# abalakrishna123/recovery-rl

Measured on AMD Instinct MI355X. Metric: env-steps/sec + SAC grad-steps/sec, Navigation1 4096 envs, 1/2/4/8 GPU, higher is better.
Workload: dtype f32

## Files before the change

include/rrl_hip.h:

```cpp
#ifndef RRL_HIP_H
#define RRL_HIP_H

#include <stdint.h>

#ifdef __cplusplus
extern "C" {
#endif

#define RRL_OK 0
#define RRL_EINVAL (-1)
#define RRL_ELAUNCH (-2)
#define RRL_ECAPTURE (-5)
#define RRL_EPLANS (-6)
#define RRL_ERANGE (-3)

enum { RRL_ENV_NAV1 = 0, RRL_ENV_NAV2 = 1, RRL_ENV_MAZE = 2 };

enum {
    RRL_STREAM_STEP = 0,
    RRL_STREAM_RESET = 1,
    RRL_STREAM_OFFLINE = 2,
    RRL_STREAM_SAMPLE = 3,
    RRL_STREAM_SAMPLE_NEG = 4,
    RRL_STREAM_CEM = 5,
// ... 181 lines not shown
    uint8_t* active;
    float* action;
} rrl_cem_set_t;
int rrl_cem_begin(const rrl_cem_set_t* s, void* stream);
int rrl_cem_finish(const rrl_cem_set_t* s, void* stream);

int rrl_gemm_f32(int mode, int G, int M, int N, int K, const float* A, int lda, long long sA,
                 const float* B, int ldb, long long sB, float* C, int ldc, long long sC,
                 const float* bias, long long sBias, int relu, const float* mask, int ldmask,
                 long long sMask, float* colsum, long long sColsum, int accumulate, void* stream);

int rrl_mlp3_forward(int G, int M, int H, int din, int dout, const float* x, int ldx, const float* W1,
                     const float* b1, const float* W2, const float* b2, const float* W3, const float* b3,
                     float* h1, float* h2, float* out, float* scratch, int finalize, void* stream);
int rrl_mlp3_is_split(int M, int H);

enum { RRL_LOSS_SAC_CRITIC = 0, RRL_LOSS_SAC_POLICY = 1, RRL_LOSS_QRISK_CRITIC = 2, RRL_LOSS_QRISK_POLICY = 3,
       RRL_LOSS_GAUSS_HEAD = 4, RRL_LOSS_STOCH_HEAD = 5, RRL_LOSS_DGD_QRISK = 6 };
typedef struct {
    int kind;
    int n_part;
    long long part_stride;
    const float *out, *out_t;
    const float *v0, *v1, *v2, *v3;
    const float* alpha;
    float f0;
    int ld, n_heads;
    long long head_stride;
    const float* d_action;
    float* loss;
    int da_parts;
    long long da_part_stride;
    int da_group;
} rrl_loss_t;

typedef struct {
    int G, M, H, din, dout, ldx;
    const float *x, *W1, *b1, *W2, *b2, *W3, *b3;
    float *h1, *h2, *out, *scratch;
    rrl_policy_head_t in_head;
    int use_in_head;
    const float* W2p;
} rrl_stack_t;
typedef struct {
    rrl_loss_t loss;
    int G, B, H, dout;
    const float *h2, *W3;
    float *dW3, *db3;
    float* dh2;
} rrl_head_bwd_t;
typedef struct {
    const float *x, *W1;
    int ldx, din;
    float* first_part;
    long long first_stride;
    float* dx_part;
    int dx_fold;
} rrl_first_layer_t;
typedef struct {
    int G, B, H;
    const float *dh2, *h1, *W2;
    float *dW2, *db2;
    float* dh1;
    rrl_first_layer_t first;
} rrl_hidden_bwd_t;
typedef struct {
    int G, B, H, din, ldx;
    const float *dh1, *x, *W1;
    float *dW1, *db1;
    float* dx;
} rrl_input_bwd_t;
int rrl_mlp3_forward_multi(int n, const rrl_stack_t* stacks, void* stream);
typedef struct {
    const rrl_draw_ahead_t* select;
    const rrl_draw_ahead_t* gather;
    const rrl_draw_t* second;
    long long noise_pairs;
    uint64_t noise_seed, noise_counter;
    uint64_t* noise_counter_dev;
    uint64_t noise_counter_inc;
    float* noise_out;
} rrl_fwd_riders_t;
int rrl_mlp3_forward_riders(const rrl_stack_t* stack, const rrl_fwd_riders_t* riders, void* stream);
int rrl_mlp_head_backward_multi(int n, const rrl_head_bwd_t* members, void* stream);
int rrl_mlp_hidden_backward_multi(int n, const rrl_hidden_bwd_t* members, void* stream);
int rrl_mlp_input_backward_multi(int n, const rrl_input_bwd_t* members, void* stream);
int rrl_mlp_backward_pair_multi(int n, const rrl_head_bwd_t* heads, const rrl_hidden_bwd_t* hidden, void* stream);

int rrl_loss_dout(const rrl_loss_t* loss, int B, float* dout, void* stream);
typedef struct {
    int B;
    const float* z;
    int n_part;
    long long part_stride;
    const float* lambda;
    float* penalty;
    float* mean;
} rrl_penalty_args_t;
int rrl_rcpo_penalty(const rrl_penalty_args_t* a, void* stream);
int rrl_policy_heads_fwd_multi(int n, const rrl_policy_head_t* heads, void* stream);
#define RRL_ADAM_MAX_SEGS 12
typedef struct {
    long long n;
    float* p;
    const float* g;
    float* m;
    float* v;
    uint64_t* step_dev;
    float* target;
    float tau;
    float weight_decay;
    const float* g2;
    const float* g_part;
    int n_part;
    long long part_stride, part_elems;
    float* w2p;
    float* target_w2p;
    long long w2_off;
    int w2_heads;
} rrl_adam_seg_t;
int rrl_adam_step_multi(int n_seg, const rrl_adam_seg_t* segs, float lr, float beta1, float beta2, float eps,
                        void* stream);
#define RRL_ADAM_MAX_DUALS 4
typedef struct {
    float *log_p, *exp_avg, *exp_avg_sq, *step;
    float* value;
    const float* stat;
    float eps_safe;
    float lr;
    const float* loss_in;
    float* loss_out;
    float f_loss;
} rrl_dual_t;
int rrl_adam_step_multi_duals(int n_seg, const rrl_adam_seg_t* segs, int n_dual, const rrl_dual_t* duals, float lr,
                              float beta1, float beta2, float eps, void* stream);
int rrl_w2_pack(int G, int H, const float* W2, float* W2p, void* stream);
int rrl_normal_fill(long long n_pairs, uint64_t seed, uint64_t counter, uint64_t* counter_dev, uint64_t counter_inc,
                    float* out, void* stream);
int rrl_recovery_select(int N, const float* z, float eps_safe, const float* task_action, int ld_task,
                        const float* rec_action, float* real_action, uint8_t* recovery, float* task_out,
                        void* stream);

#define RRL_EPLOG_I32 6
typedef struct {
    int32_t* rec_i32;
    double* rec_f64;
    int64_t cap;
    int64_t* state;
} rrl_episode_log_t;

int rrl_episode_log_append(int64_t n, const float* reward, const uint8_t* constraint, const uint8_t* success,
                           const uint8_t* ep_done, const uint8_t* recovery, int32_t* ep_len, double* ep_ret,
                           int32_t* ep_viol, int32_t* ep_rec, const rrl_episode_log_t* log, void* stream);

typedef struct {
    int hq, he, n_nets;
    const float *q_w1, *q_b1, *q_w2, *q_b2, *q_w3, *q_b3;
    const float *e_w0, *e_b0, *e_w1, *e_b1, *e_w2, *e_b2, *e_w3, *e_b3;
    const float *inputs_mu, *inputs_sigma, *max_logvar, *min_logvar;
} rrl_plan_weights_t;

int rrl_plan_supported(int hq, int he, int n_nets, int npart, int d_obs, int d_act);
long long rrl_plan_pack_floats(int hq, int he, int n_nets);
long long rrl_plan_scratch_floats(int n_nets, long long M, int pop);
int rrl_plan_pack(const rrl_plan_weights_t* w, int f16x3, float* packed, void* stream);
typedef struct {
    const float* packed;
    int hq, he, n_nets, npart;
    int f16x3;
    long long M;
// ... 195 lines not shown
```

recovery_rl_amd/_lib.py:

```python
import ctypes as C
import os
import subprocess

_HERE = os.path.dirname(os.path.abspath(__file__))
CSRC = os.path.join(_HERE, "csrc")
SO_PATH = os.environ.get("RRL_HIP_LIB") or os.path.join(CSRC, "librrl_hip.so")
INCLUDE = os.path.join(os.path.dirname(_HERE), "include")

HIP_SOURCES = ["nav_kernels.hip", "replay_kernels.hip", "maze_kernels.hip", "cem_kernels.hip",
               "mlp_kernels.hip", "mlp_fwd_kernels.hip", "update_kernels.hip", "log_kernels.hip", "plan_kernels.hip", "ens_train_kernels.hip",
               "ens_train_big_kernels.hip", "sqrl_kernels.hip", "qsample_kernels.hip", "eval_kernels.hip",
               "sqrl_f16x3_kernels.hip", "qsample_f16x3_kernels.hip"]
HIPCC_FLAGS = ["--offload-arch=gfx950", "-O3", "-std=c++17", "-fPIC", "-shared",
               "-ffp-contract=off", "-Wall", "-Wno-unused-function",
               "-Wno-bitwise-instead-of-logical"]

SOURCE_FLAGS = {
    "nav_kernels.hip": ["-mllvm", "-amdgpu-atomic-optimizer-strategy=None"],
    "maze_kernels.hip": ["-mllvm", "-amdgpu-atomic-optimizer-strategy=None"],
    "update_kernels.hip": ["-mllvm", "-amdgpu-atomic-optimizer-strategy=None"],
}

EXPORTS = [
    "rrl_abi_version", "rrl_last_hip_error", "rrl_counter_add",
    "rrl_nav_step", "rrl_nav_step_compact", "rrl_nav_reset", "rrl_nav_rollout", "rrl_nav_offline_rollouts",
    "rrl_nav_offline",
    "rrl_maze_step", "rrl_maze_reset", "rrl_maze_offline",
    "rrl_replay_push", "rrl_sample_multi", "rrl_draw_select", "rrl_mlp3_forward_riders",
    "rrl_nav_step_push_x", "rrl_maze_step_push_x",
    "rrl_sample_multi_packed", "rrl_pack_clear", "rrl_mlp3_forward_multi_packed", "rrl_mlp_head_backward_multi_packed",
    "rrl_mlp_hidden_backward_multi_packed", "rrl_mlp_backward_pair_multi_packed", "rrl_adam_step_multi_packed", "rrl_nav_step_push_packed",
    "rrl_maze_step_push_packed",
    "rrl_adam_step_multi_duals_packed", "rrl_rcpo_penalty_packed", "rrl_policy_heads_fwd_multi_packed",
    "rrl_cem_sample", "rrl_cem_update", "rrl_cem_begin", "rrl_cem_finish",
    "rrl_gemm_f32", "rrl_mlp3_forward", "rrl_mlp3_is_split",
    "rrl_mlp3_forward_multi", "rrl_mlp_head_backward_multi", "rrl_mlp_hidden_backward_multi",
    "rrl_mlp_input_backward_multi", "rrl_mlp_backward_pair_multi", "rrl_policy_heads_fwd_multi",
    "rrl_loss_dout", "rrl_rcpo_penalty", "rrl_adam_step_multi_duals",
    "rrl_adam_step_multi", "rrl_w2_pack", "rrl_normal_fill", "rrl_recovery_select", "rrl_episode_log_append",
    "rrl_plan_supported", "rrl_plan_pack_floats", "rrl_plan_scratch_floats", "rrl_plan_pack", "rrl_plan_cost",
    "rrl_ens_train_supported", "rrl_ens_scratch_floats", "rrl_ens_train_grad", "rrl_ens_train_epoch",
    "rrl_ens_train_big_supported", "rrl_ens_big_scratch_floats", "rrl_ens_train_grad_big", "rrl_ens_train_epoch_big",
    "rrl_sqrl_scratch_floats", "rrl_sqrl_act", "rrl_sqrl_act_packed",
    "rrl_qsample_scratch_floats", "rrl_qsample_act", "rrl_qsample_act_gated", "rrl_qsample_act_packed",
    "rrl_eval_rollout", "rrl_eval_rollout_packed", "rrl_eval_rollout_maze", "rrl_eval_rollout_maze_packed",
    "rrl_eval_rollout_qs", "rrl_eval_rollout_qs_packed",
    "rrl_eval_rollout_sqrl", "rrl_eval_rollout_sqrl_packed",
    "rrl_w2_pack_f16x3", "rrl_sqrl_act_f16x3", "rrl_sqrl_act_f16x3_packed",
    "rrl_qsample_act_f16x3", "rrl_qsample_act_gated_f16x3", "rrl_qsample_act_f16x3_packed",
    "rrl_eval_rollout_qs_f16x3", "rrl_eval_rollout_qs_f16x3_packed",
    "rrl_eval_rollout_sqrl_f16x3", "rrl_eval_rollout_sqrl_f16x3_packed",
]

class RRLError(RuntimeError):
    pass


def _sources():
    return [os.path.join(CSRC, f) for f in HIP_SOURCES if os.path.exists(os.path.join(CSRC, f))]


def _stale():
    if not os.path.exists(SO_PATH):
        return True
    t = os.path.getmtime(SO_PATH)
    deps = _sources() + [os.path.join(CSRC, f) for f in os.listdir(CSRC) if f.endswith(".hpp")]
    deps.append(os.path.join(INCLUDE, "rrl_hip.h"))
    return any(os.path.getmtime(d) > t for d in deps)


_FLAG_PROBES = {}


def flags_supported(hipcc, flags):
    key = (hipcc,) + tuple(flags)
    if key not in _FLAG_PROBES:
        import tempfile
        with tempfile.TemporaryDirectory() as tmp:
            src = os.path.join(tmp, "probe.hip")
            open(src, "w").write("// empty\n")
            r = subprocess.run([hipcc, "--offload-arch=gfx950", "-c", "-o", os.path.join(tmp, "probe.o"), src] + list(flags),
                               capture_output=True)
            _FLAG_PROBES[key] = r.returncode == 0
    return _FLAG_PROBES[key]


def build(force=False, verbose=False, jobs=None):
    if not force and not _stale():
        return SO_PATH
    from concurrent.futures import ThreadPoolExecutor
    hipcc = os.environ.get("HIPCC", "/opt/rocm/bin/hipcc")
    objdir = os.path.join(CSRC, "_build")
    os.makedirs(objdir, exist_ok=True)
    headers = [os.path.join(CSRC, f) for f in os.listdir(CSRC) if f.endswith(".hpp")] + [os.path.join(INCLUDE, "rrl_hip.h")]
    newest_header = max(os.path.getmtime(h) for h in headers)
    compile_flags = [f for f in HIPCC_FLAGS if f != "-shared"]

    def compile_one(src):
        obj = os.path.join(objdir, os.path.basename(src)[:-4] + ".o")
        if not force and os.path.exists(obj) and os.path.getmtime(obj) > max(os.path.getmtime(src), newest_header):
            return obj
        extra = SOURCE_FLAGS.get(os.path.basename(src), [])
        if extra and not flags_supported(hipcc, extra):
            extra = []
        cmd = [hipcc] + compile_flags + extra + ["-I", INCLUDE, "-c", "-o", obj, src]
        if verbose:
            print(" ".join(cmd))
        subprocess.check_call(cmd)
        return obj

    with ThreadPoolExecutor(max_workers=jobs or min(4, os.cpu_count() or 1)) as pool:
# ... 169 lines not shown


class rrl_sqrl_act_t(C.Structure):
    _fields_ = [(n, C.c_int) for n in ("n", "k", "H", "d_obs", "d_act")] + [
        ("obs", C.c_void_p), ("head", C.c_void_p), ("n_part", C.c_int), ("part_stride", C.c_longlong)] + [
        (n, C.c_void_p) for n in ("scale", "bias", "W1", "b1", "W2p", "b2", "W3", "b3")] + [
        ("eps_safe", C.c_float), ("seed", C.c_uint64), ("counter", C.c_uint64), ("counter_dev", C.c_void_p),
        ("counter_inc", C.c_uint64)] + [
        (n, C.c_void_p) for n in ("eps_in", "u_in", "scratch", "action", "q", "logp", "cand", "z", "pick", "cstar", "n_safe")]


STREAM_QSAMPLE = 11


class rrl_qsample_act_t(C.Structure):
    _fields_ = [(n, C.c_int) for n in ("n", "k", "H", "d_obs", "d_act")] + [
        (n, C.c_void_p) for n in ("obs", "mask", "lo", "hi", "W1", "b1", "W2p", "b2", "W3", "b3")] + [
        ("seed", C.c_uint64), ("counter", C.c_uint64), ("counter_dev", C.c_void_p), ("counter_inc", C.c_uint64)] + [
        (n, C.c_void_p) for n in ("cand_in", "scratch", "action", "q", "z", "cand", "pick")]


class rrl_qsample_gate_t(C.Structure):
    _fields_ = [("z", C.c_void_p), ("n_part", C.c_int), ("part_stride", C.c_longlong), ("eps_safe", C.c_float),
                ("task_action", C.c_void_p), ("ld_task", C.c_int), ("task_out", C.c_void_p), ("recovery_out", C.c_void_p)]


STREAM_EVAL = 12
ENV_NAV1, ENV_NAV2, ENV_MAZE = 0, 1, 2


class rrl_eval_rollout_t(C.Structure):
    _fields_ = [(n, C.c_int) for n in ("n", "T", "H", "d_obs", "d_act", "env_kind", "reset")] + [
        (n, C.c_void_p) for n in ("pos", "pW1", "pb1", "pW2p", "pb2", "pW3", "pb3", "scale", "bias",
                                  "qW1", "qb1", "qW2p", "qb2", "qW3", "qb3")] + [("eps_safe", C.c_float)] + [
        (n, C.c_void_p) for n in ("rW1", "rb1", "rW2p", "rb2", "rW3", "rb3", "rscale", "rbias", "rlog_std")] + [
        ("min_log_std", C.c_float), ("seed", C.c_uint64), ("counter", C.c_uint64)] + [
        (n, C.c_void_p) for n in ("counter_dev", "ret", "success", "violation", "steps", "tr_pos", "tr_task", "tr_real",
                                  "tr_z", "tr_eps", "tr_reward", "tr_flags")]


STREAM_EVAL_QSAMPLE = 13


class rrl_eval_rollout_qs_t(C.Structure):
    _fields_ = [("base", rrl_eval_rollout_t), ("k", C.c_int), ("horizon", C.c_int)] + [
        (n, C.c_void_p) for n in ("lo", "hi", "tr_pick", "tr_q")]


STREAM_EVAL_SQRL = 14
STREAM_EVAL_SQRL_PICK = 15


class rrl_eval_rollout_sqrl_t(C.Structure):
    _fields_ = [("base", rrl_eval_rollout_t), ("k", C.c_int), ("horizon", C.c_int)] + [
        (n, C.c_void_p) for n in ("tr_head", "tr_pick", "tr_cstar", "tr_nsafe", "tr_q")]


_lib = None


def _declare(lib):
    vp, i32, i64, u64, ci, f64, f32, ll = (C.c_void_p, C.c_int32, C.c_int64, C.c_uint64, C.c_int, C.c_double,
                                          C.c_float, C.c_longlong)
    rp = C.POINTER(rrl_replay_t)
    sig = {
        "rrl_abi_version": (ci, []),
        "rrl_last_hip_error": (ci, []),
        "rrl_counter_add": (ci, [vp, u64, vp]),
        "rrl_nav_step": (ci, [ci, i64, vp, vp, vp, u64, u64, vp, u64, vp, vp, vp, vp, vp, vp, vp,
                              vp, i32, ci, vp]),
        "rrl_nav_step_compact": (ci, [ci, i64, vp, vp, vp, u64, u64, vp, u64, vp, vp, vp, vp, i32, ci, vp]),
        "rrl_nav_reset": (ci, [ci, i64, vp, vp, vp, vp, vp, u64, u64, vp, vp]),
        "rrl_nav_rollout": (ci, [ci, i64, i32, vp, vp, u64, u64, vp, vp, vp, vp, vp, vp]),
        "rrl_nav_offline_rollouts": (i64, [ci, i64]),
        "rrl_nav_offline": (ci, [ci, i64, u64, vp, vp, vp, vp, vp, i64, vp, vp, vp]),
        "rrl_maze_step": (ci, [i64, vp, vp, u64, u64, vp, u64, vp, vp, vp, vp, vp, vp, vp, vp, i32, ci, vp]),
        "rrl_maze_reset": (ci, [i64, vp, vp, vp, vp, ci, ci, u64, u64, vp, vp]),
        "rrl_maze_offline": (ci, [i64, u64, vp, vp, vp, vp, vp, i64, vp]),
        "rrl_replay_push": (ci, [rp, i64, vp, vp, vp, vp, vp, vp, vp, vp]),
        "rrl_sample_multi": (ci, [C.POINTER(rrl_draw_t), C.POINTER(rrl_draw_t), ll, u64, u64, vp, u64, vp, vp]),
        "rrl_mlp3_forward_multi": (ci, [ci, C.POINTER(rrl_stack_t), vp]),
        "rrl_draw_select": (ci, [C.POINTER(rrl_draw_ahead_t), vp]),
        "rrl_mlp3_forward_riders": (ci, [C.POINTER(rrl_stack_t), C.POINTER(rrl_fwd_riders_t), vp]),
        "rrl_mlp_head_backward_multi": (ci, [ci, C.POINTER(rrl_head_bwd_t), vp]),
        "rrl_mlp_hidden_backward_multi": (ci, [ci, C.POINTER(rrl_hidden_bwd_t), vp]),
        "rrl_mlp_input_backward_multi": (ci, [ci, C.POINTER(rrl_input_bwd_t), vp]),
        "rrl_mlp_backward_pair_multi": (ci, [ci, C.POINTER(rrl_head_bwd_t), C.POINTER(rrl_hidden_bwd_t), vp]),
        "rrl_policy_heads_fwd_multi": (ci, [ci, C.POINTER(rrl_policy_head_t), vp]),
        "rrl_sample_multi_packed": (ci, [ci, C.POINTER(rrl_sample_args_t), vp]),
        "rrl_pack_clear": (ci, []),
        "rrl_mlp3_forward_multi_packed": (ci, [ci, C.POINTER(ci), C.POINTER(C.POINTER(rrl_stack_t)), vp]),
        "rrl_mlp_head_backward_multi_packed": (ci, [ci, C.POINTER(ci), C.POINTER(C.POINTER(rrl_head_bwd_t)), vp]),
        "rrl_mlp_hidden_backward_multi_packed": (ci, [ci, C.POINTER(ci), C.POINTER(C.POINTER(rrl_hidden_bwd_t)), vp]),
        "rrl_mlp_backward_pair_multi_packed": (ci, [ci, C.POINTER(ci), C.POINTER(C.POINTER(rrl_head_bwd_t)),
                                                    C.POINTER(C.POINTER(rrl_hidden_bwd_t)), vp]),
        "rrl_adam_step_multi_packed": (ci, [ci, C.POINTER(ci), C.POINTER(C.POINTER(rrl_adam_seg_t)), C.POINTER(f32), f32,
                                            f32, f32, vp]),
        "rrl_adam_step_multi_duals_packed": (ci, [ci, C.POINTER(ci), C.POINTER(C.POINTER(rrl_adam_seg_t)), C.POINTER(ci),
                                                  C.POINTER(C.POINTER(rrl_dual_t)), C.POINTER(f32), f32, f32, f32, vp]),
        "rrl_rcpo_penalty_packed": (ci, [ci, C.POINTER(rrl_penalty_args_t), vp]),
        "rrl_policy_heads_fwd_multi_packed": (ci, [ci, C.POINTER(ci), C.POINTER(C.POINTER(rrl_policy_head_t)), vp]),
        "rrl_nav_step_push_packed": (ci, [ci, ci, C.POINTER(rrl_step_push_t), vp]),
        "rrl_maze_step_push_packed": (ci, [ci, C.POINTER(rrl_step_push_t), vp]),
        "rrl_nav_step_push_x": (ci, [ci, C.POINTER(rrl_step_push_t), vp]),
        "rrl_maze_step_push_x": (ci, [C.POINTER(rrl_step_push_t), vp]),
        "rrl_cem_sample": (ci, [C.POINTER(rrl_cem_t), vp]),
        "rrl_cem_update": (ci, [C.POINTER(rrl_cem_t), vp]),
        "rrl_cem_begin": (ci, [C.POINTER(rrl_cem_set_t), vp]),
        "rrl_cem_finish": (ci, [C.POINTER(rrl_cem_set_t), vp]),
        "rrl_gemm_f32": (ci, [ci, ci, ci, ci, ci, vp, ci, C.c_longlong, vp, ci, C.c_longlong, vp, ci,
                              C.c_longlong, vp, C.c_longlong, ci, vp, ci, C.c_longlong, vp, C.c_longlong,
                              ci, vp]),
        "rrl_mlp3_forward": (ci, [ci, ci, ci, ci, ci, vp, ci, vp, vp, vp, vp, vp, vp, vp, vp, vp, vp, ci, vp]),
        "rrl_mlp3_is_split": (ci, [ci, ci]),
        "rrl_loss_dout": (ci, [C.POINTER(rrl_loss_t), ci, vp, vp]),
        "rrl_rcpo_penalty": (ci, [C.POINTER(rrl_penalty_args_t), vp]),
        "rrl_adam_step_multi_duals": (ci, [ci, C.POINTER(rrl_adam_seg_t), ci, C.POINTER(rrl_dual_t), f32, f32, f32, f32, vp]),
        "rrl_adam_step_multi": (ci, [ci, C.POINTER(rrl_adam_seg_t), f32, f32, f32, f32, vp]),
        "rrl_w2_pack": (ci, [ci, ci, vp, vp, vp]),
        "rrl_normal_fill": (ci, [ll, u64, u64, vp, u64, vp, vp]),
        "rrl_recovery_select": (ci, [ci, vp, f32, vp, ci, vp, vp, vp, vp, vp]),
        "rrl_plan_supported": (ci, [ci, ci, ci, ci, ci, ci]),
        "rrl_plan_pack_floats": (ll, [ci, ci, ci]),
        "rrl_plan_scratch_floats": (ll, [ci, ll, ci]),
        "rrl_plan_pack": (ci, [C.POINTER(rrl_plan_weights_t), ci, vp, vp]),
        "rrl_plan_cost": (ci, [C.POINTER(rrl_plan_cost_t), vp]),
        "rrl_ens_train_supported": (ci, [ci, ci, ci, ci]),
        "rrl_ens_scratch_floats": (ll, [ci]),
        "rrl_ens_train_epoch": (ci, [C.POINTER(rrl_ens_t), ci, C.POINTER(rrl_adam_seg_t), f32, f32, f32, f32, vp, vp,
                                     vp, ll, ll, ci, vp, vp, vp]),
        "rrl_ens_train_grad": (ci, [C.POINTER(rrl_ens_t), ci, vp, vp, vp, ll, vp, vp, vp]),
        "rrl_ens_train_big_supported": (ci, [ci, ci, ci]),
        "rrl_ens_big_scratch_floats": (ll, [ci, ll]),
        "rrl_ens_train_grad_big": (ci, [C.POINTER(rrl_ens_t), ll, vp, vp, vp, ll, vp, vp, vp]),
        "rrl_ens_train_epoch_big": (ci, [C.POINTER(rrl_ens_t), ci, C.POINTER(rrl_adam_seg_t), f32, f32, f32, f32, vp, vp,
                                         vp, ll, ll, ll, vp, vp, vp]),
        "rrl_sqrl_scratch_floats": (ll, [ll, ci]),
        "rrl_sqrl_act": (ci, [C.POINTER(rrl_sqrl_act_t), vp]),
        "rrl_sqrl_act_packed": (ci, [ci, C.POINTER(rrl_sqrl_act_t), vp]),
        "rrl_w2_pack_f16x3": (ci, [ci, ci, vp, vp, vp]),
        "rrl_sqrl_act_f16x3": (ci, [C.POINTER(rrl_sqrl_act_t), vp]),
        "rrl_sqrl_act_f16x3_packed": (ci, [ci, C.POINTER(rrl_sqrl_act_t), vp]),
        "rrl_qsample_scratch_floats": (ll, [ll, ci]),
        "rrl_qsample_act": (ci, [C.POINTER(rrl_qsample_act_t), vp]),
        "rrl_qsample_act_gated": (ci, [C.POINTER(rrl_qsample_act_t), C.POINTER(rrl_qsample_gate_t), vp]),
        "rrl_qsample_act_packed": (ci, [ci, C.POINTER(rrl_qsample_act_t), C.POINTER(rrl_qsample_gate_t), vp]),
        "rrl_qsample_act_f16x3": (ci, [C.POINTER(rrl_qsample_act_t), vp]),
        "rrl_qsample_act_gated_f16x3": (ci, [C.POINTER(rrl_qsample_act_t), C.POINTER(rrl_qsample_gate_t), vp]),
        "rrl_qsample_act_f16x3_packed": (ci, [ci, C.POINTER(rrl_qsample_act_t), C.POINTER(rrl_qsample_gate_t), vp]),
        "rrl_eval_rollout": (ci, [C.POINTER(rrl_eval_rollout_t), vp]),
        "rrl_eval_rollout_packed": (ci, [ci, C.POINTER(rrl_eval_rollout_t), vp]),
        "rrl_eval_rollout_maze": (ci, [C.POINTER(rrl_eval_rollout_t), ci, vp]),
        "rrl_eval_rollout_maze_packed": (ci, [ci, C.POINTER(rrl_eval_rollout_t), C.POINTER(ci), vp]),
        "rrl_eval_rollout_qs": (ci, [C.POINTER(rrl_eval_rollout_qs_t), vp]),
        "rrl_eval_rollout_qs_packed": (ci, [ci, C.POINTER(rrl_eval_rollout_qs_t), vp]),
        "rrl_eval_rollout_sqrl": (ci, [C.POINTER(rrl_eval_rollout_sqrl_t), vp]),
        "rrl_eval_rollout_sqrl_packed": (ci, [ci, C.POINTER(rrl_eval_rollout_sqrl_t), vp]),
        "rrl_eval_rollout_qs_f16x3": (ci, [C.POINTER(rrl_eval_rollout_qs_t), vp, vp]),
        "rrl_eval_rollout_qs_f16x3_packed": (ci, [ci, C.POINTER(rrl_eval_rollout_qs_t), C.POINTER(vp), vp]),
        "rrl_eval_rollout_sqrl_f16x3": (ci, [C.POINTER(rrl_eval_rollout_sqrl_t), vp, vp]),
        "rrl_eval_rollout_sqrl_f16x3_packed": (ci, [ci, C.POINTER(rrl_eval_rollout_sqrl_t), C.POINTER(vp), vp]),
        "rrl_episode_log_append": (ci, [i64, vp, vp, vp, vp, vp, vp, vp, vp, vp, C.POINTER(rrl_episode_log_t), vp]),
    }
    for name, (res, args) in sig.items():
        fn = getattr(lib, name)
        fn.restype = res
# ... 53 lines not shown
```

recovery_rl_amd/csrc/mlp_fwd_kernels.hip:

```cpp
#include "mlp_common.hpp"
#include "replay_draw.hpp"

namespace {

using rrl_host::check_launch;


struct StackArgs {
    const float* x;
    const float* W1; const float* b1;
    const float* W2; const float* b2;
    const float* W3; const float* b3;
    float* h1; float* h2;
    float* out;
    int M, H, din, dout, ldx;
    rrl_policy_head_t in_head;
    int use_in_head;
    const float* W2p;
};

constexpr int kStackRows = 16;
constexpr int kStackMaxH = 256;

using rrl::row16_sum;
// ... 55 lines not shown
#pragma unroll
        for (int t = 0; t < R; ++t) {
            acc0[t] = f32x4{0.f, 0.f, 0.f, 0.f};
            acc1[t] = f32x4{0.f, 0.f, 0.f, 0.f};
        }
#pragma unroll
        for (int j = 0; j < kStackMaxH / 16; ++j) {
            if (16 * j < H) {
#pragma unroll
                for (int t = 0; t < R; ++t) {
                    const float4 av = *reinterpret_cast<const float4*>(h1s + (16 * t + i) * ldh + 4 * q + 16 * j);
                    acc0[t] = __builtin_amdgcn_mfma_f32_16x16x4f32(av.x, wv[j].x, acc0[t], 0, 0, 0);
                    acc1[t] = __builtin_amdgcn_mfma_f32_16x16x4f32(av.y, wv[j].y, acc1[t], 0, 0, 0);
                    acc0[t] = __builtin_amdgcn_mfma_f32_16x16x4f32(av.z, wv[j].z, acc0[t], 0, 0, 0);
                    acc1[t] = __builtin_amdgcn_mfma_f32_16x16x4f32(av.w, wv[j].w, acc1[t], 0, 0, 0);
                }
            }
        }
#pragma unroll
        for (int t = 0; t < R; ++t) {
            const f32x4 acc = acc0[t] + acc1[t];
#pragma unroll
            for (int r = 0; r < 4; ++r) {
                const int rr = 16 * t + 4 * q + r;
                float v = acc[r] + bias2;
                v = v > 0.f ? v : 0.f;
                h2s[rr * ldh + n0 + i] = v;
                if (a.h2 && m0 + rr < a.M) a.h2[((long long)g * a.M + m0 + rr) * H + n0 + i] = v;
            }
        }
    }
    __syncthreads();
#pragma unroll
    for (int t = 0; t < R; ++t) {
        const int r = 16 * t + wave;
        float v = 0.f;
#pragma unroll
        for (int it = 0; it < kStackMaxH / 16; ++it)
            if (i + 16 * it < H) v = fmaf(h2s[r * ldh + i + 16 * it], w3v[it], v);
        v = row16_sum(v);
        if (i == 0 && q < a.dout && m0 + r < a.M) a.out[((long long)g * a.M + m0 + r) * a.dout + q] = v + bias3;
    }
}

template <int R>
__global__ __launch_bounds__(1024) void mlp3_fwd_kernel(StackArgs a) {
    __shared__ __attribute__((aligned(16))) float h1s[R * kStackRows * (kStackMaxH + 20)];
    __shared__ __attribute__((aligned(16))) float h2s[R * kStackRows * (kStackMaxH + 20)];
    mlp3_fwd_body<R>(a, blockIdx.x, blockIdx.y, h1s, h2s);
}

__device__ __forceinline__ void globalize(StackArgs& a) {
    rrl_pack::to_global_all(a.x, a.W1, a.b1, a.W2, a.b2, a.W3, a.b3, a.h1, a.h2, a.out, a.W2p);
    rrl_pack::globalize(a.in_head);
}
struct StackGroup {
    StackArgs a[kMaxGroup];
    float* partial[kMaxGroup];
    int G[kMaxGroup], tiles[kMaxGroup];
    int nb[kMaxGroup];
    int first[kMaxGroup + 1];
    int n;
};

template <int R>
__global__ __launch_bounds__(1024) void mlp3_fwd_group_kernel(StackGroup sg) {
    __shared__ __attribute__((aligned(16))) float h1s[R * kStackRows * (kStackMaxH + 20)];
    __shared__ __attribute__((aligned(16))) float h2s[R * kStackRows * (kStackMaxH + 20)];
    int k = 0;
    while (k + 1 < sg.n && (int)blockIdx.x >= sg.first[k + 1]) ++k;
    const int local = blockIdx.x - sg.first[k];
    mlp3_fwd_body<R>(sg.a[k], local % sg.tiles[k], local / sg.tiles[k], h1s, h2s);
}

constexpr int kSplit = 4;
constexpr int kSplitPad = 20;

struct RowKeys {
    const uint32_t* keys;
    const float* lo; const float* hi;
    int B;
    uint32_t last;
};

template <int R, int HC, bool LOOP = false, bool KEYED = false>
__device__ __forceinline__ void mlp3_fwd_split_body(const StackArgs& a, float* partial, int bx, int g, int z, int G,
                                                    float* h1s, float* h2s, int nb = 1, int tiles = 1, float* xs_own = nullptr,
                                                    const RowKeys* rk = nullptr) {
    const int tid = threadIdx.x, lane = tid & 63;
    const int wave = __builtin_amdgcn_readfirstlane(tid >> 6);
    constexpr int kW = 4;
    const int H = HC ? HC : a.H, ldh = H + kSplitPad, HS = H / kSplit, ld2 = HS + 1;
    constexpr int kJ = HC ? HC / 16 : kStackMaxH / 16;
    constexpr int kU = HC ? HC / (16 * kW) : kStackMaxH / (16 * kW);
    constexpr int kT3 = HC ? HC / (16 * kSplit) : kStackMaxH / (16 * kSplit);
    const int colbase = z * HS;
    const int M = a.M, din = a.din, dout = a.dout;
    const float* W1 = a.W1 + (long long)g * H * din;
    const float* b1 = a.b1 + (long long)g * H;
    const float* W2 = a.W2 + (long long)g * H * H;
    const float* b2 = a.b2 + (long long)g * H;
    const float* W3 = a.W3 + (long long)g * dout * H;
    const float* b3 = a.b3 + (long long)g * dout;
    const int ntiles1 = H / 16;
    const bool has_tile2 = HC ? true : wave * 16 < HS;
    const int n2 = colbase + (has_tile2 ? wave * 16 : 0);

    float w1b[kU], bias1[kU];
    float4 wv[kJ];
    float bias2, w3v[kT3], bias3;
    const auto load_weights = [&]() {
        const int i = lane & 15, q = lane >> 4, o3 = min(q, dout - 1);
#pragma unroll
        for (int u = 0; u < kU; ++u) {
            const int t = min(wave + kW * u, ntiles1 - 1);
            const float wv1 = W1[(t * 16 + i) * din + min(q, din - 1)];
            w1b[u] = (q < din) ? wv1 : 0.f;
            bias1[u] = b1[t * 16 + i];
        }
        if (HC == 256) {
            const bool frag = a.W2p != nullptr;
            const char* wbase = frag ? reinterpret_cast<const char*>(a.W2p + (long long)g * H * H) + (n2 / 16) * (kJ * 1024)
                                     : reinterpret_cast<const char*>(W2 + (long long)n2 * H);
            rrl_pack::to_global(wbase);
            const unsigned voff = frag ? unsigned(lane) * 16u : unsigned(i * H + 4 * q) * 4u;
            const unsigned stepb = frag ? 1024u : 64u;
#pragma unroll
            for (int j = 0; j < kJ; ++j) wv[j] = *reinterpret_cast<const float4*>(wbase + j * stepb + voff);
        } else {
            const float* wrow = W2 + (long long)(n2 + i) * H + 4 * q;
#pragma unroll
            for (int j = 0; j < kJ; ++j) wv[j] = *reinterpret_cast<const float4*>(wrow + min(16 * j, H - 16));
        }
        bias2 = b2[n2 + i];
#pragma unroll
        for (int it = 0; it < kT3; ++it) w3v[it] = W3[o3 * H + colbase + min(i + 16 * it, HS - 1)];
        const float b3v = b3[o3];
        bias3 = (z == 0) ? b3v : 0.f;
    };
    if (LOOP) load_weights();
    const int blk0 = LOOP ? bx * nb : bx, blk1 = LOOP ? min(blk0 + nb, tiles) : bx + 1;
    const auto load_x = [&](int blk, float (&x)[R]) {
        const int i = lane & 15, q = lane >> 4, m0 = blk * (R * kStackRows);
        if (KEYED && rk->keys) {
            const float* lo = rk->lo;
            const float* hi = rk->hi;
            rrl_pack::to_global_all(lo, hi);
#pragma unroll
            for (int t = 0; t < R; ++t) {
                const int m = m0 + min(16 * t + i, M - 1 - m0);
                const bool upper = m >= rk->B;
                const unsigned e = 2u * min(rk->keys[upper ? m - rk->B : m], rk->last) + unsigned(min(q, din - 1));
                const float v_lo = lo[e], v_hi = hi[e];
                x[t] = upper ? v_hi : v_lo;
            }
            return;
        }
        const float* const xblk = a.x + (long long)m0 * a.ldx;
#pragma unroll
        for (int t = 0; t < R; ++t) x[t] = xblk[unsigned(min(16 * t + i, M - 1 - m0) * a.ldx + min(q, din - 1))];
    };
    struct HeadOps { float e, mp[4], rp[4], ob; };
    const int head_wave = (bx + g + z) & (kW - 1);
    const auto load_head = [&](int blk, HeadOps& o) {
        const rrl_policy_head_t& hd = a.in_head;
        const int m0 = blk * (R * kStackRows), j = lane & 1;
        const int rb = min(min(lane >> 1, R * kStackRows - 1), M - 1 - m0);
        const unsigned row = unsigned(m0 + rb), xoff = unsigned(rb * a.ldx);
        const float* const xblk = a.x + (long long)m0 * a.ldx;
        const float* eb = hd.eps ? hd.eps : xblk;
        const float* obb = hd.obs_in ? hd.obs_in : xblk;
        rrl_pack::to_global_all(eb, obb);
        o.e = eb[hd.eps ? 2 * row + j : xoff];
        const bool gauss = hd.kind == RRL_HEAD_GAUSS;
        const unsigned im = gauss ? 4 * row + j : 2 * row + j, ir = gauss ? im + 2 : im;
#pragma unroll
        for (int k = 0; k < 4; ++k) {
            const float* const hk = hd.head + min(k, hd.n_part - 1) * hd.part_stride;
            o.mp[k] = hk[im];
            o.rp[k] = hk[ir];
        }
        o.ob = obb[hd.obs_in ? 2 * row + j : xoff + j];
    };
    const int li = lane & 15, lq = lane >> 4;
    float* const h1w = h1s + (4 * lq) * ldh + wave * 16 + li;
    const float* const h1r = h1s + li * ldh + 4 * lq;
    float* const h2w = h2s + (4 * lq) * ld2 + wave * 16 + li;
    const float* const h3r = h2s + (wave * 4) * ld2 + li;
    const unsigned g1off = unsigned((4 * lq) * H + wave * 16 + li);
    const unsigned g2off = unsigned((4 * lq) * H + n2 + li);
    float xn[R];
    HeadOps hn;
    if (LOOP) {
        load_x(blk0, xn);
        if (a.use_in_head && wave == head_wave) load_head(blk0, hn);
    }
    for (int blk = blk0; blk < blk1; ++blk) {
    int m0 = blk * (R * kStackRows);
    if (LOOP) asm volatile("" : "+s"(m0));
    int lane_b = lane;
    if (LOOP) asm volatile("" : "+v"(lane_b));
    const int i = lane_b & 15, q = lane_b >> 4;
    float* const h1g = (a.h1 && z == 0) ? a.h1 + ((long long)g * M + m0) * H : nullptr;
    float* const h2g = a.h2 ? a.h2 + ((long long)g * M + m0) * H : nullptr;
    float* const pout = partial + (((long long)z * G + g) * M + m0) * dout;
    const bool full = m0 + R * kStackRows <= M;
    const int last = M - 1 - m0;

    float xa[R];
    if (LOOP) {
#pragma unroll
        for (int t = 0; t < R; ++t) xa[t] = xn[t];
        load_x(min(blk + 1, blk1 - 1), xn);
    } else load_x(blk, xa);
    if (a.use_in_head) {
        static_assert(R * kStackRows <= 32, "the input head is ONE pass of one wave, a lane per (row, action dimension): 32 rows");
        const rrl_policy_head_t& hd = a.in_head;
        const bool writer = z == 0 && g == 0;
        float* xs = LOOP ? xs_own : h2s;
        if (wave == head_wave) {
            const int rl = min(lane_b >> 1, R * kStackRows - 1), j = lane_b & 1;
            const bool lane_ok = (lane_b >> 1) < R * kStackRows;
            const unsigned row = unsigned(m0 + min(rl, last));
            const bool row_ok = lane_ok && rl <= last;
            const bool gauss = hd.kind == RRL_HEAD_GAUSS;
            const float sc = hd.scale[j], bi = hd.bias[j];
// ... 163 lines not shown
__global__ __launch_bounds__(256, 4) void mlp3_fwd_split_kernel(StackArgs a, float* partial) {
    extern __shared__ __attribute__((aligned(16))) float lds[];
    float* h2s = R > 1 ? lds : lds + R * kStackRows * (kStackMaxH + kSplitPad);
    if (a.H == 256) mlp3_fwd_split_body<R, 256>(a, partial, blockIdx.x, blockIdx.y, blockIdx.z, gridDim.y, lds, h2s);
    else mlp3_fwd_split_body<R, 0>(a, partial, blockIdx.x, blockIdx.y, blockIdx.z, gridDim.y, lds, h2s);
}

template <int R>
__global__ __launch_bounds__(256, 4) void mlp3_fwd_split_group_kernel(StackGroup sg) {
    extern __shared__ __attribute__((aligned(16))) float lds[];
    const int k = blockIdx.y;
    StackArgs a = sg.a[k];
    float* partial = sg.partial[k];
    const int G = sg.G[k], tiles = sg.tiles[k];
    globalize(a);
    rrl_pack::to_global(partial);
    arrive_together(a.M, a.H, a.din, a.dout, a.ldx, a.use_in_head, a.in_head.kind, a.in_head.n_part, a.in_head.part_stride,
                    a.in_head.ld_action, a.in_head.min_log_std, G, tiles);
    const int local = blockIdx.x;
    if (local >= tiles * G * kSplit) return;
    const int bx = local % tiles, rest = local / tiles;
    float* h2s = R > 1 ? lds : lds + R * kStackRows * (kStackMaxH + kSplitPad);
    if (a.H == 256) mlp3_fwd_split_body<R, 256>(a, partial, bx, rest % G, rest / G, G, lds, h2s);
    else mlp3_fwd_split_body<R, 0>(a, partial, bx, rest % G, rest / G, G, lds, h2s);
}

__global__ __launch_bounds__(256, 4) void mlp3_fwd_split_flat_group_kernel(StackGroup sg) {
    extern __shared__ __attribute__((aligned(16))) float lds[];
    arrive_together(sg.first[1], sg.first[2], sg.first[3]);
    const int x = blockIdx.x;
    const int k = (x >= sg.first[1]) + (x >= sg.first[2]) + (x >= sg.first[3]);
    StackArgs a = sg.a[k];
    float* partial = sg.partial[k];
    const int G = sg.G[k], tiles = sg.tiles[k];
    globalize(a);
    rrl_pack::to_global(partial);
    arrive_together(a.M, a.H, a.din, a.dout, a.ldx, a.use_in_head, a.in_head.kind, a.in_head.n_part, a.in_head.part_stride,
                    a.in_head.ld_action, a.in_head.min_log_std, G, tiles);
    const int local = x - sg.first[k];
    const int bx = local % tiles, rest = local / tiles;
    if (a.M <= kSplitSmallM)
        mlp3_fwd_split_body<1, 256>(a, partial, bx, rest % G, rest / G, G, lds, lds + kStackRows * (kStackMaxH + kSplitPad));
    else
        mlp3_fwd_split_body<kBigR, 256>(a, partial, bx, rest % G, rest / G, G, lds, lds);
}

struct FwdRiders {
    DrawArgs sel;
    long long rows_ahead;
    uint32_t* sel_keys;
    DrawArgs gat;
    const uint32_t* gat_keys;
    DrawArgs second;
    NoiseArgs nz;
    int slot_sel, slot_gat, slot_second, slot_noise;
    int n;
};

template <int R>
__global__ __launch_bounds__(256, 4) void mlp3_fwd_split_riders_kernel(StackArgs a, float* partial, int G, int tiles, RowKeys rk,
                                                                       FwdRiders rd) {
    extern __shared__ __attribute__((aligned(16))) float lds[];
    const int x = blockIdx.x;
    if (x < rd.n) {
        char* smem = reinterpret_cast<char*>(lds);
        if (x == rd.slot_sel)
            select_ahead_body(rd.sel.rb, rd.sel.B, rd.sel.seed, rd.sel.counter, rd.sel.counter_dev, rd.sel.table_mask,
                              rd.rows_ahead, rd.sel_keys, smem);
        else if (x == rd.slot_gat)
            gather_ahead_body(rd.gat.rb, rd.gat.B, rd.gat.counter, rd.gat.counter_dev, rd.gat.counter_inc, rd.gat_keys,
                              rd.gat.out);
        else if (x == rd.slot_second) draw_body(rd.second, smem);
        else noise_body(rd.nz, x - rd.slot_noise);
        return;
    }
    arrive_together(a.M, a.H, a.din, a.dout, a.ldx, a.use_in_head, a.in_head.kind, a.in_head.n_part, a.in_head.part_stride,
                    a.in_head.ld_action, a.in_head.min_log_std, G, tiles, rk.B, rk.last);
    const int local = x - rd.n;
    const int bx = local % tiles, rest = local / tiles;
    float* h2s = R > 1 ? lds : lds + R * kStackRows * (kStackMaxH + kSplitPad);
    mlp3_fwd_split_body<R, 256, false, true>(a, partial, bx, rest % G, rest / G, G, lds, h2s, 1, 1, nullptr, &rk);
}

template <int R>
__global__ __launch_bounds__(256, 4) void mlp3_fwd_split_pack_kernel(const StackGroup* __restrict__ groups, rrl_pack::Idx ix) {
    extern __shared__ __attribute__((aligned(16))) float lds[];
    RRL_PACK_LOCATE(ix, groups, s, local);
    const StackGroup& sg = groups[s];
    const int k = blockIdx.y;
    StackArgs a = sg.a[k];
    float* partial = sg.partial[k];
    const int G = sg.G[k], tiles = sg.tiles[k];
    globalize(a);
    rrl_pack::to_global(partial);
    arrive_together(a.M, a.H, a.din, a.dout, a.ldx, a.use_in_head, a.in_head.kind, a.in_head.n_part, a.in_head.part_stride,
                    a.in_head.ld_action, a.in_head.min_log_std, G, tiles);
    if (local >= tiles * G * kSplit) return;
    const int bx = local % tiles, rest = local / tiles;
    float* h2s = R > 1 ? lds : lds + R * kStackRows * (kStackMaxH + kSplitPad);
    if (a.H == 256) mlp3_fwd_split_body<R, 256>(a, partial, bx, rest % G, rest / G, G, lds, h2s);
    else mlp3_fwd_split_body<R, 0>(a, partial, bx, rest % G, rest / G, G, lds, h2s);
}

#ifndef RRL_FWD_LOOP_WAVES
#define RRL_FWD_LOOP_WAVES 3
#endif
template <int R>
__global__ __launch_bounds__(256, RRL_FWD_LOOP_WAVES) void mlp3_fwd_split_pack_loop_kernel(const StackGroup* __restrict__ groups, rrl_pack::Idx ix) {
    extern __shared__ __attribute__((aligned(16))) float lds[];
    RRL_PACK_LOCATE(ix, groups, s, local);
    const StackGroup& sg = groups[s];
    const int k = blockIdx.y;
    StackArgs a = sg.a[k];
    float* partial = sg.partial[k];
    const int G = sg.G[k], tiles = sg.tiles[k], nb = sg.nb[k];
    globalize(a);
    rrl_pack::to_global(partial);
    arrive_together(a.M, a.H, a.din, a.dout, a.ldx, a.use_in_head, a.in_head.kind, a.in_head.n_part, a.in_head.part_stride,
                    a.in_head.ld_action, a.in_head.min_log_std, G, tiles, nb);
    const int wt = (tiles + nb - 1) / nb;
    if (local >= wt * G * kSplit) return;
    const int bx = local % wt, rest = local / wt;
    float* h2s = lds + R * kStackRows * (kStackMaxH + kSplitPad);
    float* xs = h2s + R * kStackRows * (kStackMaxH / kSplit + 1);
    mlp3_fwd_split_body<R, 256, true>(a, partial, bx, rest % G, rest / G, G, lds, h2s, nb, tiles, xs);
}

__global__ void sum_partials_kernel(int n, const float* __restrict__ partial, float* __restrict__ out) {
    const int e = blockIdx.x * blockDim.x + threadIdx.x;
    if (e >= n) return;
    float v = partial[e];
#pragma unroll
    for (int z = 1; z < kSplit; ++z) v += partial[(long long)z * n + e];
    out[e] = v;
}

constexpr int kPackSmallR2MinSeeds = 3;
constexpr int kResidentWorkgroups = 256 * RRL_FWD_LOOP_WAVES;
constexpr int kLoopMaxBlocks = 32, kLoopMinBlocks = 8;

static int env_int_fwd(const char* name, int fallback) {
    const char* v = getenv(name);
    return v && *v ? atoi(v) : fallback;
}
static bool pack_fwd_loop() {
    static const bool on = env_int_fwd("RRL_PACK_FWD_LOOP", 1) != 0;
    return on;
}

}

extern "C" {

int rrl_mlp3_is_split(int M, int H) {
    (void)M;
    return ((H % (16 * kSplit)) == 0 && H <= kStackMaxH) ? kSplit : 0;
}

static int stack_check(int G, int M, int H, int din, int dout, const float* x, const float* W1, const float* b1,
                       const float* W2, const float* b2, const float* W3, const float* b3, const float* out) {
    if (!x || !W1 || !b1 || !W2 || !b2 || !W3 || !b3 || !out) return RRL_EINVAL;
    if (G <= 0 || G > 65535 || M <= 0 || din <= 0 || din > 4 || dout <= 0 || dout > 4) return RRL_ERANGE;
    if (H <= 0 || H > kStackMaxH || (H % 16) != 0) return RRL_ERANGE;
    return RRL_OK;
}

// ... 35 lines not shown
    if (!st || n <= 0 || n > kMaxGroup) return RRL_EINVAL;
    sg = StackGroup{};
    sg.n = n;
    sg.first[0] = 0;
    path = -1;
    bool any_big = false, all_split256 = true;
    for (int k = 0; k < n; ++k) {
        const bool split = st[k].scratch && rrl_mlp3_is_split(st[k].M, st[k].H);
        all_split256 = all_split256 && split && st[k].H == 256;
        any_big = any_big || (split && st[k].H == 256 && st[k].M > kSplitSmallM);
    }
    bool any_small = false;
    for (int k = 0; k < n; ++k) any_small = any_small || st[k].M <= kSplitSmallM;
    const bool mixed = any_big && any_small && all_split256;
    if (mixed && !flat) small_r = big_r;
    for (int k = 0; k < n; ++k) {
        const rrl_stack_t& p = st[k];
        const int rc = stack_check(p.G, p.M, p.H, p.din, p.dout, p.x, p.W1, p.b1, p.W2, p.b2, p.W3, p.b3, p.out);
        if (rc != RRL_OK) return rc;
        sg.a[k] = StackArgs{p.x, p.W1, p.b1, p.W2, p.b2, p.W3, p.b3, p.h1, p.h2, p.out, p.M, p.H, p.din, p.dout, p.ldx,
                            p.in_head, p.use_in_head, p.H == 256 ? p.W2p : nullptr};
        if (sg.a[k].W2p && (reinterpret_cast<uintptr_t>(p.W2p) & 15)) return RRL_EINVAL;
        if (p.use_in_head) {
            const rrl_policy_head_t& h = p.in_head;
            if (p.din != 4 || !h.head || !h.scale || !h.bias || h.n_part <= 0 || h.n_part > 4 ||
                (h.kind == RRL_HEAD_GAUSS ? !h.eps : (h.kind != RRL_HEAD_STOCH || !h.log_std)) || (h.obs_out && !h.action))
                return RRL_EINVAL;
            if (!(p.scratch && rrl_mlp3_is_split(p.M, p.H))) return RRL_EINVAL;
            if (h.kind == RRL_HEAD_STOCH) sg.a[k].in_head.obs_out = nullptr;
        }
        sg.partial[k] = p.scratch;
        sg.G[k] = p.G;
        sg.nb[k] = 1;
        int my;
        const long long tiles16 = (p.M + kStackRows - 1) / kStackRows;
        if (p.scratch && rrl_mlp3_is_split(p.M, p.H)) {
            my = (p.M <= kSplitSmallM || p.H != 256) ? 0 : 3;
            if (my == 0 && small_r > 1 && p.H != 256) return RRL_EINVAL;
            const int rows = (my == 0 ? small_r : big_r) * kStackRows;
            if (mixed) my = 5;
            sg.tiles[k] = (p.M + rows - 1) / rows;
            sg.nb[k] = loop_nb < sg.tiles[k] ? loop_nb : sg.tiles[k];
            sg.first[k + 1] = sg.first[k] + (sg.tiles[k] + sg.nb[k] - 1) / sg.nb[k] * p.G * kSplit;
        } else if (tiles16 * p.G > 256) {
            my = 2;
            sg.tiles[k] = (p.M + 2 * kStackRows - 1) / (2 * kStackRows);
            sg.first[k + 1] = sg.first[k] + sg.tiles[k] * p.G;
        } else {
            my = 1;
            sg.tiles[k] = int(tiles16);
            sg.first[k + 1] = sg.first[k] + sg.tiles[k] * p.G;
        }
        if (path >= 0 && my != path) return RRL_EINVAL;
        path = my;
    }
    for (int k = n; k < kMaxGroup; ++k) sg.first[k + 1] = sg.first[n];
    return RRL_OK;
}

int rrl_mlp3_forward_multi(int n, const rrl_stack_t* st, void* stream) {
    StackGroup sg;
    int path;
    const int rc = build_stack_group(n, st, sg, path);
    if (rc != RRL_OK) return rc;
    hipStream_t s = (hipStream_t)stream;
    const int most = largest_member(sg, n);
    if (path == 0) {
        hipLaunchKernelGGL(mlp3_fwd_split_group_kernel<1>, dim3(most, n), dim3(256), split_lds_floats(1) * 4, s, sg);
    } else if (path == 3) {
        static const bool ok = grant_lds((const void*)mlp3_fwd_split_group_kernel<kBigR>, split_lds_floats(kBigR) * 4);
        if (!ok) return RRL_ERANGE;
        hipLaunchKernelGGL(mlp3_fwd_split_group_kernel<kBigR>, dim3(most, n), dim3(256),
                           split_lds_floats(kBigR) * 4, s, sg);
    } else if (path == 5) {
        constexpr size_t lds_floats = split_lds_floats(kBigR) > split_lds_floats(1) ? split_lds_floats(kBigR) : split_lds_floats(1);
        static const bool ok = grant_lds((const void*)mlp3_fwd_split_flat_group_kernel, lds_floats * 4);
        if (!ok) return RRL_ERANGE;
        hipLaunchKernelGGL(mlp3_fwd_split_flat_group_kernel, dim3(sg.first[n]), dim3(256), lds_floats * 4, s, sg);
    } else if (path == 1) hipLaunchKernelGGL((mlp3_fwd_group_kernel<1>), dim3(sg.first[n]), dim3(1024), 0, s, sg);
    else hipLaunchKernelGGL((mlp3_fwd_group_kernel<2>), dim3(sg.first[n]), dim3(1024), 0, s, sg);
    return check_launch();
}

int rrl_mlp3_forward_riders(const rrl_stack_t* stack, const rrl_fwd_riders_t* riders, void* stream) {
    if (!stack || !riders) return RRL_EINVAL;
    StackGroup sg;
    int path;
    int rc = build_stack_group(1, stack, sg, path);
    if (rc != RRL_OK) return rc;
    if ((path != 0 && path != 3) || stack->H != 256) return RRL_EINVAL;
    FwdRiders rd{};
    RowKeys rk{};
    rd.slot_sel = rd.slot_gat = rd.slot_second = rd.slot_noise = -1;
    size_t lds = split_lds_floats(path == 0 ? 1 : kBigR) * 4;
    const auto rider = [&](const rrl_draw_t* d, DrawArgs& a, int& slot) {
        int threads = 0;
        size_t l = 0;
        const int r = draw_setup(*d, a, threads, l);
        if (r != RRL_OK) return r;
        if (threads > 256) return int(RRL_ERANGE);
        lds = l > lds ? l : lds;
        slot = rd.n++;
        return int(RRL_OK);
    };
    if (riders->select) {
        const rrl_draw_ahead_t& s = *riders->select;
        if (!s.draw || !s.keys || s.rows_ahead < 0 || s.draw->stratified != RRL_DRAW_UNIFORM) return RRL_EINVAL;
        if ((rc = rider(s.draw, rd.sel, rd.slot_sel)) != RRL_OK) return rc;
        rd.rows_ahead = s.rows_ahead;
        rd.sel_keys = s.keys;
    }
    if (riders->gather) {
        const rrl_draw_ahead_t& s = *riders->gather;
        if (!s.draw || !s.keys || s.draw->stratified != RRL_DRAW_UNIFORM) return RRL_EINVAL;
        if ((rc = rider(s.draw, rd.gat, rd.slot_gat)) != RRL_OK) return rc;
        rd.gat_keys = s.keys;
        if (stack->M != 2 * rd.gat.B || stack->din != 2 || stack->use_in_head) return RRL_EINVAL;
        rk = RowKeys{s.keys, rd.gat.rb.s2, rd.gat.rb.s, rd.gat.B, uint32_t(rd.gat.rb.cap - 1)};
    }
    if (riders->second && (rc = rider(riders->second, rd.second, rd.slot_second)) != RRL_OK) return rc;
    if (riders->noise_pairs < 0 || riders->noise_pairs >= (1LL << 32) || (riders->noise_pairs > 0 && !riders->noise_out))
        return RRL_EINVAL;
    if (riders->noise_pairs > 0) {
        rd.nz = NoiseArgs{riders->noise_pairs, riders->noise_seed, riders->noise_counter, riders->noise_counter_dev,
                          riders->noise_counter_inc, riders->noise_out, 0};
        noise_blocks(rd.nz, 256);
        rd.slot_noise = rd.n;
        rd.n += rd.nz.blocks;
    }
    if (lds > 64 * 1024) return RRL_ERANGE;
    const dim3 grid(unsigned(rd.n + sg.first[1]));
    hipStream_t s = (hipStream_t)stream;
    if (path == 0)
        hipLaunchKernelGGL(mlp3_fwd_split_riders_kernel<1>, grid, dim3(256), lds, s, sg.a[0], sg.partial[0], sg.G[0],
                           sg.tiles[0], rk, rd);
    else
        hipLaunchKernelGGL(mlp3_fwd_split_riders_kernel<kBigR>, grid, dim3(256), lds, s, sg.a[0], sg.partial[0], sg.G[0],
                           sg.tiles[0], rk, rd);
    return check_launch();
}

int rrl_mlp3_forward_multi_packed(int S, const int* n, const rrl_stack_t* const* members, void* stream) {
    rrl_pack::Key key(rrl_pack::Site::StackForward, S);
    if (!key.groups(S, n, members, kMaxGroup)) return RRL_EINVAL;
    if (S == 1) {
        StackGroup sg;
        int path;
        const int rc = build_stack_group(n[0], members[0], sg, path);
        if (rc != RRL_OK) return rc;
        if (path != 0 && path != 3 && path != 5) return RRL_EINVAL;
        return rrl_mlp3_forward_multi(n[0], members[0], stream);
    }
    hipStream_t st = (hipStream_t)stream;
    const rrl_pack::Plan* plan = rrl_pack::lookup(key);
    if (!plan) {
        std::vector<StackGroup> groups(S);
        int path = -1;
        const int big_r = kBigR;
        bool all256 = true;
        for (int s = 0; s < S; ++s)
            for (int k = 0; k < n[s]; ++k) all256 = all256 && members[s] && members[s][k].H == 256;
        const int small_r = (S >= kPackSmallR2MinSeeds && all256) ? big_r : 1;
        int loop_nb = 1;
        const auto build_all = [&]() {
            path = -1;
            for (int s = 0; s < S; ++s) {
                int my;
                const int r = build_stack_group(n[s], members[s], groups[s], my, big_r, small_r, loop_nb, false);
                if (r != RRL_OK) return r;
                if (my == 5) my = 3;
                if ((my != 0 && my != 3) || (path >= 0 && my != path)) return int(RRL_EINVAL);
                path = my;
            }
            return int(RRL_OK);
        };
        int rc = build_all();
        if (rc != RRL_OK) return rc;
        if (path == 3 && all256 && pack_fwd_loop()) {
            const int share = rrl_pack::seed_share(S);
            const auto fits = [&]() {
                long long all = 0;
                for (int s = 0; s < S; ++s) {
                    all += groups[s].first[n[s]];
                    if (share > 1 && (long long)groups[s].first[n[s]] * share > kResidentWorkgroups) return false;
                }
                return all <= kResidentWorkgroups;
            };
            while (!fits() && loop_nb < kLoopMaxBlocks) {
                ++loop_nb;
                rc = build_all();
                if (rc != RRL_OK) return rc;
            }
            if (loop_nb < kLoopMinBlocks) {
                loop_nb = 1;
                rc = build_all();
                if (rc != RRL_OK) return rc;
            }
        }
        if (path == 3 || (small_r > 1 && path == 0)) {
            static const bool ok = grant_lds((const void*)mlp3_fwd_split_pack_kernel<kBigR>, split_lds_floats(kBigR) * 4);
            static const bool ok2 = grant_lds((const void*)mlp3_fwd_split_pack_loop_kernel<kBigR>, loop_lds_floats(kBigR) * 4);
            if (!ok || !ok2) return RRL_ERANGE;
            path = loop_nb > 1 ? 4 : 3;
        }
        int most[rrl_pack::kMaxSeeds], members_most = 1;
        for (int s = 0; s < S; ++s) {
            most[s] = largest_member(groups[s], n[s]);
            members_most = n[s] > members_most ? n[s] : members_most;
        }
        rrl_pack::Launch l = rrl_pack::place_members(S, most);
        l.i0 = path;
        l.i1 = members_most;
        plan = rrl_pack::publish(key, groups, l, st);
        if (!plan) return rrl_pack::store_error();
    }
    if (plan->i0 == 0)
        hipLaunchKernelGGL(mlp3_fwd_split_pack_kernel<1>, dim3(plan->grid, plan->i1), dim3(256), split_lds_floats(1) * 4, st,
                           (const StackGroup*)plan->dev, plan->ix);
    else if (plan->i0 == 4)
        hipLaunchKernelGGL(mlp3_fwd_split_pack_loop_kernel<kBigR>, dim3(plan->grid, plan->i1), dim3(256),
                           loop_lds_floats(kBigR) * 4, st, (const StackGroup*)plan->dev, plan->ix);
// ... 8 lines not shown
```

recovery_rl_amd/csrc/mlp_kernels.hip:

```cpp
#include <hip/hip_runtime.h>

#include <stdlib.h>

#include <algorithm>

#include "mlp_common.hpp"

namespace {

using rrl_host::check_launch;
using rrl::row16_sum;

constexpr int kTile = 16;
constexpr int kPanel = 128;
constexpr int kLd = 20;
constexpr int kVec = 8;

struct GemmArgs {
    const float* A;
    const float* B;
    float* C;
    const float* bias;
    const float* mask;
    float* colsum;
    int M, N, K;
    int lda, ldb, ldc, ldmask;
    long long sA, sB, sC, sBias, sMask, sColsum;
    int relu;
    int accumulate;
    const float* x;
    const float* W1;
    float* first_part;
    float* dx_part;
    long long first_stride;
    int ldx, din, G;
    int skip_c;
    int dx_fold;
};

__device__ __forceinline__ void globalize(GemmArgs& a) {
    rrl_pack::to_global_all(a.A, a.B, a.C, a.bias, a.mask, a.colsum, a.x, a.W1, a.first_part, a.dx_part);
}

template <int VEC>
struct FragT {
    float4 v[VEC];
};
using Frag = FragT<kVec>;

template <bool FAST>
__device__ __forceinline__ float4 load4(const float* __restrict__ base, long long row_off, int k, int K,
                                        bool row_ok) {
    if (FAST) return *reinterpret_cast<const float4*>(base + row_off + k);
    float v[4];
#pragma unroll
    for (int t = 0; t < 4; ++t) {
        const int kk = min(k + t, K - 1);
        const float x = base[row_off + (kk < 0 ? 0 : kk)];
        v[t] = (row_ok && k + t < K) ? x : 0.f;
    }
    return make_float4(v[0], v[1], v[2], v[3]);
}

template <bool FAST, int VEC>
__device__ __forceinline__ void load_direct(FragT<VEC>& f, const float* __restrict__ src, int ld, int row0,
                                            int rows, int k0, int K, int lane) {
    const int gr = row0 + (lane & 15);
    const bool ok = gr < rows;
    const long long off = (long long)(ok ? gr : rows - 1) * ld;
#pragma unroll
    for (int j = 0; j < VEC; ++j) f.v[j] = load4<FAST>(src, off, k0 + 16 * j + 4 * (lane >> 4), K, ok);
}

template <bool FAST, int VEC>
__device__ __forceinline__ void load_staged(FragT<VEC>& f, const float* __restrict__ src, int ld, int col0,
                                            int cols, int k0, int K, int lane) {
    const int c = col0 + (lane & 3) * 4;
#pragma unroll
    for (int j = 0; j < VEC; ++j) {
        const int k = k0 + (lane >> 2) + 16 * j;
        const bool ok = k < K;
        f.v[j] = load4<FAST>(src, (long long)(ok ? k : K - 1) * ld, c, cols, ok);
    }
}
template <int VEC>
__device__ __forceinline__ void store_staged(const FragT<VEC>& f, float* tile, int lane) {
#pragma unroll
    for (int j = 0; j < VEC; ++j)
        *reinterpret_cast<float4*>(tile + ((lane >> 2) + 16 * j) * kLd + (lane & 3) * 4) = f.v[j];
// ... 939 lines not shown
}

__device__ __forceinline__ void head_bwd_dispatch(const HeadBwdArgs& hb, int bx, int g, float (*red)[4][kCols],
                                                  float* dsh) {
    switch (hb.la.kind) {
        case RRL_LOSS_SAC_CRITIC: head_bwd_loss_body<RRL_LOSS_SAC_CRITIC>(hb, bx, g, red, dsh); break;
        case RRL_LOSS_SAC_POLICY: head_bwd_loss_body<RRL_LOSS_SAC_POLICY>(hb, bx, g, red, dsh); break;
        case RRL_LOSS_QRISK_CRITIC: head_bwd_loss_body<RRL_LOSS_QRISK_CRITIC>(hb, bx, g, red, dsh); break;
        case RRL_LOSS_QRISK_POLICY:
        case RRL_LOSS_DGD_QRISK: head_bwd_loss_body<RRL_LOSS_QRISK_POLICY>(hb, bx, g, red, dsh); break;
        case RRL_LOSS_GAUSS_HEAD: head_bwd_loss_body<RRL_LOSS_GAUSS_HEAD>(hb, bx, g, red, dsh); break;
        case RRL_LOSS_STOCH_HEAD: head_bwd_loss_body<RRL_LOSS_STOCH_HEAD>(hb, bx, g, red, dsh); break;
        default: head_bwd_loss_body<kPlainDOut>(hb, bx, g, red, dsh); break;
    }
}

__device__ __forceinline__ void globalize(HeadBwdArgs& hb) {
    rrl_loss_t& l = hb.la;
    rrl_pack::to_global_all(l.out, l.out_t, l.v0, l.v1, l.v2, l.v3, l.alpha, l.d_action, l.loss, hb.h2, hb.W3, hb.dW3, hb.db3,
                            hb.dh2);
}
struct HeadBwdGroup {
    HeadBwdArgs p[kMaxGroup];
    int G[kMaxGroup], blocks_x[kMaxGroup];
    int first[kMaxGroup + 1];
    int n;
};

__device__ __forceinline__ void head_bwd_member_body(const HeadBwdGroup& hg, int local, float (*red)[4][kCols], float* dsh) {
    const int k = blockIdx.y;
    HeadBwdArgs hb = hg.p[k];
    const int blocks_x = hg.blocks_x[k], G = hg.G[k];
    globalize(hb);
    const rrl_loss_t& l = hb.la;
    arrive_together(hb.B, hb.H, hb.dout, hb.need_w, l.kind, l.n_part, l.part_stride, l.f0, l.ld, l.n_heads, l.head_stride,
                    l.da_parts, l.da_part_stride, l.da_group, blocks_x, G);
    if (local >= blocks_x * G) return;
    head_bwd_dispatch(hb, local % blocks_x, local / blocks_x, red, dsh);
}

__global__ __launch_bounds__(256) void head_bwd_group_kernel(HeadBwdGroup hg) {
    __shared__ float red[kSlices][4][kCols];
    __shared__ float dsh[1024 * 4];
    head_bwd_member_body(hg, blockIdx.x, red, dsh);
}

__global__ __launch_bounds__(256) void head_bwd_pack_kernel(const HeadBwdGroup* __restrict__ groups, rrl_pack::Idx ix) {
    __shared__ float red[kSlices][4][kCols];
    __shared__ float dsh[1024 * 4];
    RRL_PACK_LOCATE(ix, groups, s, local);
    head_bwd_member_body(groups[s], local, red, dsh);
}

constexpr int kPairPanel = 64;
constexpr int kPairTileFloats = 2 * kPairPanel * kLd;
struct PairJobs {
    HiddenJob job[kMaxGroup][2];
    HeadBwdArgs head[kMaxGroup];
    int blocks_x[kMaxGroup];
};
template <int DOUT>
__device__ __forceinline__ void pair_eval_dout(const rrl_loss_t& la, int B, int g, float* dsh, int b0, int nb) {
    float unused[2] = {0.f, 0.f};
    if constexpr (DOUT == 4) {
        eval_dout_rows<RRL_LOSS_GAUSS_HEAD>(la, B, g, dsh, unused, b0, nb);
    } else if constexpr (DOUT == 2) {
        eval_dout_rows<RRL_LOSS_STOCH_HEAD>(la, B, g, dsh, unused, b0, nb);
    } else {
        switch (la.kind) {
            case RRL_LOSS_SAC_CRITIC: eval_dout_rows<RRL_LOSS_SAC_CRITIC>(la, B, g, dsh, unused, b0, nb); break;
            case RRL_LOSS_SAC_POLICY: eval_dout_rows<RRL_LOSS_SAC_POLICY>(la, B, g, dsh, unused, b0, nb); break;
            case RRL_LOSS_QRISK_CRITIC: eval_dout_rows<RRL_LOSS_QRISK_CRITIC>(la, B, g, dsh, unused, b0, nb); break;
            default: eval_dout_rows<RRL_LOSS_QRISK_POLICY>(la, B, g, dsh, unused, b0, nb); break;
        }
    }
}
constexpr int kPairDsh = 1024;
template <int DOUT>
constexpr int pair_smem_floats() {
    return 4 * kPairTileFloats + kPairDsh + (DOUT > 1 ? DOUT * 256 : 0);
}

template <int DOUT>
__device__ __forceinline__ void backward_pair_body(const PairJobs& pj, int x, float* smem) {
    const int k = blockIdx.y, z = blockIdx.z;
    HeadBwdArgs hb = pj.head[k];
    const int blocks_x = pj.blocks_x[k];
    globalize(hb);
    const rrl_loss_t& l = hb.la;
    if (z == 2) {
        const int G = pj.job[k][0].G;
        arrive_together(hb.B, hb.H, hb.dout, hb.need_w, l.kind, l.n_part, l.part_stride, l.f0, l.ld, l.n_heads, l.head_stride,
                        l.da_parts, l.da_part_stride, l.da_group, blocks_x, G);
        const int local = x;
        if (local >= blocks_x * G) return;
        float (*red)[4][kCols] = reinterpret_cast<float (*)[4][kCols]>(smem);
        const int bx = local % blocks_x, g = local / blocks_x;
        if constexpr (DOUT == 4) {
            head_bwd_loss_body<RRL_LOSS_GAUSS_HEAD>(hb, bx, g, red, smem + 1024);
        } else if constexpr (DOUT == 2) {
            head_bwd_loss_body<RRL_LOSS_STOCH_HEAD>(hb, bx, g, red, smem + 1024);
        } else {
            switch (l.kind) {
                case RRL_LOSS_SAC_CRITIC: head_bwd_loss_body<RRL_LOSS_SAC_CRITIC>(hb, bx, g, red, smem + 1024); break;
                case RRL_LOSS_SAC_POLICY: head_bwd_loss_body<RRL_LOSS_SAC_POLICY>(hb, bx, g, red, smem + 1024); break;
                case RRL_LOSS_QRISK_CRITIC: head_bwd_loss_body<RRL_LOSS_QRISK_CRITIC>(hb, bx, g, red, smem + 1024); break;
                default: head_bwd_loss_body<RRL_LOSS_QRISK_POLICY>(hb, bx, g, red, smem + 1024); break;
            }
        }
        return;
    }
    HiddenJob j = pj.job[k][z];
    GemmArgs& ga = j.ga;
    globalize(ga);
    arrive_together(ga.M, ga.N, ga.K, ga.lda, ga.ldb, ga.ldc, ga.ldmask, ga.sA, ga.sB, ga.sC, ga.sMask, ga.sColsum,
                    ga.relu, ga.accumulate, ga.first_stride, ga.ldx, ga.din, ga.G, ga.skip_c, ga.dx_fold, j.tiles, j.tiles_x, j.G,
                    hb.B, hb.H, l.kind, l.n_part, l.part_stride, l.f0, l.ld, l.n_heads, l.head_stride, l.da_parts, l.da_part_stride,
                    l.da_group);
    const int t0 = 4 * x;
    if (t0 >= j.tiles * j.G) return;
    const int g = t0 / j.tiles;
    float* dsh = smem + 4 * kPairTileFloats;
    float* w3s = dsh + kPairDsh;
    const float* w3 = hb.W3 + (long long)g * DOUT * hb.H;
    const int wave = threadIdx.x >> 6, t = t0 + wave - g * j.tiles;
    const int row_tile = (t0 - g * j.tiles) / j.tiles_x;
    const auto eval_dout = [&]() {
        if constexpr (DOUT > 1) {
            for (int e = threadIdx.x; e < DOUT * hb.H; e += 256) w3s[e] = w3[e];
        }
        if (z == 1) pair_eval_dout<DOUT>(l, hb.B, g, dsh, 0, hb.B);
        else pair_eval_dout<DOUT>(l, hb.B, g, dsh, row_tile * kTile, kTile);
        __syncthreads();
    };
    float* As = smem + wave * kPairTileFloats;
    float* Bs = As + kPairPanel * kLd;
    using Behind = decltype(eval_dout);
    if (z == 1)
        gemm16_tile<2, true, kPairPanel, true, true, true, Behind, DOUT, true>(ga, As, Bs, t % j.tiles_x, t / j.tiles_x, g, dsh,
                                                                               w3, eval_dout, w3s, false, nullptr, smem,
                                                                               kPairTileFloats);
    else {
        const bool fold = ga.dx_part && ga.dx_fold;
        float sx = 0.f;
        gemm16_tile<1, true, kPairPanel, true, true, true, Behind, DOUT, true>(ga, As, Bs, t % j.tiles_x, t / j.tiles_x, g, dsh,
                                                                               w3, eval_dout, w3s, fold, &sx, smem, kPairTileFloats);
        if (fold) {
            __syncthreads();
            dsh[threadIdx.x] = sx;
            __syncthreads();
            if (wave == 0) {
                const int lane = threadIdx.x, rr = lane & 15, dd = lane >> 4;
                float gs = dsh[lane];
                gs += dsh[64 + lane];
                gs += dsh[128 + lane];
                gs += dsh[192 + lane];
                const int bx = t % j.tiles_x, by = t / j.tiles_x;
                if (dd < ga.din)
                    ga.dx_part[(((long long)(bx >> 2) * ga.G + g) * ga.M + by * kTile + rr) * ga.din + dd] = gs;
            }
        }
    }
}
template <int DOUT>
__global__ __launch_bounds__(256) void backward_pair_kernel(PairJobs pj) {
    __shared__ __attribute__((aligned(16))) float smem[pair_smem_floats<DOUT>()];
    backward_pair_body<DOUT>(pj, blockIdx.x, smem);
}
template <int DOUT>
__global__ __launch_bounds__(256) void backward_pair_pack_kernel(const PairJobs* __restrict__ groups, rrl_pack::Idx ix) {
    __shared__ __attribute__((aligned(16))) float smem[pair_smem_floats<DOUT>()];
    RRL_PACK_LOCATE(ix, groups, s, local);
    backward_pair_body<DOUT>(groups[s], local, smem);
}

template <int DOUT>
constexpr int pair_block_smem_floats() {
    return BlkLds<1, 2>::kFloats + kPairDsh + DOUT * 256;
}
template <int DOUT>
__global__ __launch_bounds__(256) void backward_pair_block_pack_kernel(const PairJobs* __restrict__ groups, rrl_pack::Idx ix) {
    __shared__ __attribute__((aligned(16))) float smem[pair_block_smem_floats<DOUT>() > 5120 ? pair_block_smem_floats<DOUT>() : 5120];
    RRL_PACK_LOCATE(ix, groups, s, local);
    const PairJobs& pj = groups[s];
    const int k = blockIdx.y, z = blockIdx.z;
    HeadBwdArgs hb = pj.head[k];
    const int blocks_x = pj.blocks_x[k];
    globalize(hb);
    const rrl_loss_t& l = hb.la;
    if (z == 2) {
        const int G = pj.job[k][0].G;
        arrive_together(hb.B, hb.H, hb.dout, hb.need_w, l.kind, l.n_part, l.part_stride, l.f0, l.ld, l.n_heads, l.head_stride,
                        l.da_parts, l.da_part_stride, l.da_group, blocks_x, G);
        if (local >= blocks_x * G) return;
        float (*red)[4][kCols] = reinterpret_cast<float (*)[4][kCols]>(smem);
        const int bx = local % blocks_x, g = local / blocks_x;
        if constexpr (DOUT == 4) {
            head_bwd_loss_body<RRL_LOSS_GAUSS_HEAD>(hb, bx, g, red, smem + 1024);
        } else if constexpr (DOUT == 2) {
            head_bwd_loss_body<RRL_LOSS_STOCH_HEAD>(hb, bx, g, red, smem + 1024);
        } else {
            switch (l.kind) {
                case RRL_LOSS_SAC_CRITIC: head_bwd_loss_body<RRL_LOSS_SAC_CRITIC>(hb, bx, g, red, smem + 1024); break;
                case RRL_LOSS_SAC_POLICY: head_bwd_loss_body<RRL_LOSS_SAC_POLICY>(hb, bx, g, red, smem + 1024); break;
                case RRL_LOSS_QRISK_CRITIC: head_bwd_loss_body<RRL_LOSS_QRISK_CRITIC>(hb, bx, g, red, smem + 1024); break;
                default: head_bwd_loss_body<RRL_LOSS_QRISK_POLICY>(hb, bx, g, red, smem + 1024); break;
            }
        }
        return;
    }
    HiddenJob j = pj.job[k][z];
    GemmArgs& ga = j.ga;
    globalize(ga);
    arrive_together(ga.M, ga.N, ga.K, ga.lda, ga.ldb, ga.ldc, ga.ldmask, ga.sA, ga.sB, ga.sC, ga.sMask, ga.sColsum,
                    ga.relu, ga.accumulate, ga.first_stride, ga.ldx, ga.din, ga.G, ga.skip_c, ga.dx_fold, j.tiles, j.tiles_x, j.G,
                    hb.B, hb.H, l.kind, l.n_part, l.part_stride, l.f0, l.ld, l.n_heads, l.head_stride, l.da_parts, l.da_part_stride,
                    l.da_group);
    if (local >= j.tiles * j.G) return;
    const int g = local / j.tiles, b = local - g * j.tiles;
    float* dsh = smem + BlkLds<1, 2>::kFloats;
    float* w3s = dsh + kPairDsh;
    const float* w3 = hb.W3 + (long long)g * DOUT * hb.H;
    const auto eval_dout = [&]() {
        for (int e = threadIdx.x; e < DOUT * hb.H; e += 256) w3s[e] = w3[e];
        if (z == 1) pair_eval_dout<DOUT>(l, hb.B, g, dsh, 0, hb.B);
        else pair_eval_dout<DOUT>(l, hb.B, g, dsh, (b / j.tiles_x) * BlkLds<1, 2>::BM, BlkLds<1, 2>::BM);
        __syncthreads();
    };
    using Behind = decltype(eval_dout);
    if (z == 1) gemm_block<2, 1, 2, DOUT, Behind>(ga, smem, b % j.tiles_x, b / j.tiles_x, g, dsh, w3s, eval_dout);
    else gemm_block<1, 1, 2, DOUT, Behind>(ga, smem, b % j.tiles_x, b / j.tiles_x, g, dsh, w3s, eval_dout);
}

struct InputBwdArgs {
    int B, H, din, ldx, need_w, need_x;
    const float* dh1;
    const float* x;
    const float* W1;
    float* dW1;
    float* db1;
    float* dx;
};

__device__ __forceinline__ void input_bwd_body(const InputBwdArgs& ib, int bx, int g, float (*red)[5][kCols]) {
    const int B = ib.B, H = ib.H, din = ib.din, ldx = ib.ldx, need_w = ib.need_w, need_x = ib.need_x;
    const float* __restrict__ dh1 = ib.dh1;
    const float* __restrict__ x = ib.x;
    const float* __restrict__ W1 = ib.W1;
    float* __restrict__ dW1 = ib.dW1;
    float* __restrict__ db1 = ib.db1;
    float* __restrict__ dx = ib.dx;
    const int wblocks = need_w ? (H + kCols - 1) / kCols : 0;
    if (bx < wblocks) {
        const int hc = threadIdx.x & (kCols - 1), slice = threadIdx.x / kCols, h = bx * kCols + hc;
        const bool hok = h < H;
        const int hh = hok ? h : H - 1;
// ... 305 lines not shown
            case RRL_LOSS_GAUSS_HEAD: hipLaunchKernelGGL((head_bwd_loss_kernel<RRL_LOSS_GAUSS_HEAD>), grid, block, 0, st, hb); return;
            case RRL_LOSS_STOCH_HEAD: hipLaunchKernelGGL((head_bwd_loss_kernel<RRL_LOSS_STOCH_HEAD>), grid, block, 0, st, hb); return;
            default: break;
        }
    }
    hipLaunchKernelGGL(head_bwd_group_kernel, dim3(largest_member(hg, n), n), dim3(256), 0, st, hg);
}

int rrl_mlp_head_backward_multi(int n, const rrl_head_bwd_t* ps, void* stream) {
    HeadBwdGroup hg;
    const int rc = build_head_group(n, ps, hg);
    if (rc != RRL_OK) return rc;
    launch_head_group(hg, n, (hipStream_t)stream);
    return check_launch();
}

static bool hidden_blocks(int n, const rrl_hidden_bwd_t* ps, HiddenGroup& hg, int wm, int wn);
static int build_pair_jobs(int n, const rrl_head_bwd_t* heads, const rrl_hidden_bwd_t* hidden, PairJobs& pj, int& most, bool& pair,
                           int& dout, HeadBwdGroup* hg_out = nullptr, HiddenGroup* hd_out = nullptr, bool blocks = false) {
    HeadBwdGroup hg;
    int rc = build_head_group(n, heads, hg);
    if (rc != RRL_OK) return rc;
    HiddenGroup hd;
    rc = build_hidden_group(n, hidden, hd);
    if (rc != RRL_OK) return rc;
    if (hg_out) *hg_out = hg;
    if (hd_out) *hd_out = hd;
    pair = true;
    dout = 0;
    for (int k = 0; k < n && pair; ++k) {
        const rrl_head_bwd_t& h = heads[k];
        const rrl_hidden_bwd_t& d = hidden[k];
        const int kind = h.loss.kind;
        const int nn_tiles = hd.per_head[k] - hd.tn_tiles[k];
        const int my = ((kind >= RRL_LOSS_SAC_CRITIC && kind <= RRL_LOSS_QRISK_POLICY) || kind == RRL_LOSS_DGD_QRISK) ? 1
                       : kind == RRL_LOSS_GAUSS_HEAD ? 4 : kind == RRL_LOSS_STOCH_HEAD ? 2 : 0;
        pair = my != 0 && (dout == 0 || dout == my) && h.dout == my && h.dh2 && h.dh2 == d.dh2 &&
               h.G == d.G && h.B == d.B && h.H == d.H && h.B * my <= kPairDsh && h.H <= 256 && hd.fast[k] &&
               (h.H % kPairPanel) == 0 && (h.B % kPairPanel) == 0 && (nn_tiles % 4) == 0 && (hd.tn_tiles[k] % 4) == 0 &&
               (reinterpret_cast<uintptr_t>(h.h2) & 15) == 0 && (reinterpret_cast<uintptr_t>(h.W3) & 15) == 0;
        dout = my;
    }
    if (pair && blocks) pair = hidden_blocks(n, hidden, hd, 1, 2);
    if (!pair) return RRL_OK;
    pj = PairJobs{};
    most = 1;
    const int per_wg = blocks ? 1 : 4;
    for (int k = 0; k < n; ++k) {
        const int nn_tiles = hd.per_head[k] - hd.tn_tiles[k];
        pj.job[k][0] = HiddenJob{hd.nn[k], nn_tiles, hd.nn_tiles_x[k], 1, hidden[k].G};
        pj.job[k][1] = HiddenJob{hd.tn[k], hd.tn_tiles[k], hd.tn_tiles_x[k], 1, hidden[k].G};
        pj.job[k][0].ga.A = pj.job[k][1].ga.A = heads[k].h2;
        pj.head[k] = hg.p[k];
        pj.head[k].dh2 = nullptr;
        pj.blocks_x[k] = hg.blocks_x[k];
        most = std::max(most, std::max(std::max(hd.tn_tiles[k], nn_tiles) * hidden[k].G / per_wg, hg.blocks_x[k] * heads[k].G));
    }
    return RRL_OK;
}

int rrl_mlp_backward_pair_multi(int n, const rrl_head_bwd_t* heads, const rrl_hidden_bwd_t* hidden, void* stream) {
    PairJobs pj;
    HeadBwdGroup hg;
    HiddenGroup hd;
    int most = 1, dout = 0;
    bool pair = false;
    const int rc = build_pair_jobs(n, heads, hidden, pj, most, pair, dout, &hg, &hd);
    if (rc != RRL_OK) return rc;
    hipStream_t st = (hipStream_t)stream;
    if (!pair) {
        if (wants_fold(n, hidden)) return RRL_ERANGE;
        launch_head_group(hg, n, st);
        HiddenJobs hj;
        const int m = hidden_jobs(n, hidden, hd, hj);
        hipLaunchKernelGGL(gemm16_group_kernel, dim3(m, n, 2), dim3(64), 0, st, hj);
        return check_launch();
    }
    if (dout == 4) hipLaunchKernelGGL(backward_pair_kernel<4>, dim3(most, n, 3), dim3(256), 0, st, pj);
    else if (dout == 2) hipLaunchKernelGGL(backward_pair_kernel<2>, dim3(most, n, 3), dim3(256), 0, st, pj);
    else hipLaunchKernelGGL(backward_pair_kernel<1>, dim3(most, n, 3), dim3(256), 0, st, pj);
    return check_launch();
}

static int head_pack_plan(const rrl_pack::Key& key, int S, const int* n, const rrl_head_bwd_t* const* members, hipStream_t st,
                          const rrl_pack::Plan*& plan) {
    std::vector<HeadBwdGroup> groups(S);
    int most[rrl_pack::kMaxSeeds], members_most = 1;
    for (int s = 0; s < S; ++s) {
        const int rc = build_head_group(n[s], members[s], groups[s]);
        if (rc != RRL_OK) return rc;
        most[s] = largest_member(groups[s], n[s]);
        members_most = std::max(members_most, n[s]);
    }
    rrl_pack::Launch l = rrl_pack::place_members(S, most);
    l.i0 = members_most;
    plan = rrl_pack::publish(key, groups, l, st);
    return plan ? RRL_OK : rrl_pack::store_error();
}

int rrl_mlp_head_backward_multi_packed(int S, const int* n, const rrl_head_bwd_t* const* members, void* stream) {
    rrl_pack::Key key(rrl_pack::Site::HeadBackward, S);
    if (!key.groups(S, n, members, kMaxGroup)) return RRL_EINVAL;
    if (S == 1) return rrl_mlp_head_backward_multi(n[0], members[0], stream);
    hipStream_t st = (hipStream_t)stream;
    const rrl_pack::Plan* plan = rrl_pack::lookup(key);
    if (!plan) {
        const int rc = head_pack_plan(key, S, n, members, st, plan);
        if (rc != RRL_OK) return rc;
    }
    hipLaunchKernelGGL(head_bwd_pack_kernel, dim3(plan->grid, plan->i0), dim3(256), 0, st, (const HeadBwdGroup*)plan->dev, plan->ix);
    return check_launch();
}

int rrl_mlp_backward_pair_multi_packed(int S, const int* n, const rrl_head_bwd_t* const* heads,
                                       const rrl_hidden_bwd_t* const* hidden, void* stream) {
    rrl_pack::Key key(rrl_pack::Site::BackwardPair, S), key_head(rrl_pack::Site::HeadBackward, S),
        key_hidden(rrl_pack::Site::HiddenBackward, S);
    if (!key_head.groups(S, n, heads, kMaxGroup) || !key_hidden.groups(S, n, hidden, kMaxGroup)) return RRL_EINVAL;
    if (S == 1) return rrl_mlp_backward_pair_multi(n[0], heads[0], hidden[0], stream);
    key.add(key_head.bytes.data(), key_head.bytes.size());
    key.add(key_hidden.bytes.data(), key_hidden.bytes.size());
    hipStream_t st = (hipStream_t)stream;
    const rrl_pack::Plan* plan = rrl_pack::lookup(key);
    if (!plan) {
        std::vector<PairJobs> jobs(S);
        int most[rrl_pack::kMaxSeeds], members_most = 1;
        const bool blocks = S > pack_pair_max_seeds();
        bool pair = S <= pack_pair_block_max_seeds();
        int dout = 0;
        for (int s = 0; s < S && pair; ++s) {
            int m = 1, my = 0;
            const int rc = build_pair_jobs(n[s], heads[s], hidden[s], jobs[s], m, pair, my, nullptr, nullptr, blocks);
            if (rc != RRL_OK) return rc;
            pair = pair && (dout == 0 || dout == my);
            dout = my;
            most[s] = m;
            members_most = std::max(members_most, n[s]);
        }
        rrl_pack::Launch l;
        if (pair) {
            l = rrl_pack::place_members(S, most);
            l.i0 = members_most;
            l.i1 = dout + (blocks ? 16 : 0);
        } else {
            jobs.clear();
        }
        plan = rrl_pack::publish(key, jobs, l, st);
        if (!plan) return rrl_pack::store_error();
    }
    if (plan->i1 == 0) {
        const int rc = rrl_mlp_head_backward_multi_packed(S, n, heads, stream);
        return rc != RRL_OK ? rc : rrl_mlp_hidden_backward_multi_packed(S, n, hidden, stream);
    }
    const dim3 grid(plan->grid, plan->i0, 3);
    const PairJobs* dev = (const PairJobs*)plan->dev;
    if (plan->i1 == 16 + 4) hipLaunchKernelGGL(backward_pair_block_pack_kernel<4>, grid, dim3(256), 0, st, dev, plan->ix);
    else if (plan->i1 == 16 + 2) hipLaunchKernelGGL(backward_pair_block_pack_kernel<2>, grid, dim3(256), 0, st, dev, plan->ix);
    else if (plan->i1 == 16 + 1) hipLaunchKernelGGL(backward_pair_block_pack_kernel<1>, grid, dim3(256), 0, st, dev, plan->ix);
    else if (plan->i1 == 4) hipLaunchKernelGGL(backward_pair_pack_kernel<4>, grid, dim3(256), 0, st, dev, plan->ix);
    else if (plan->i1 == 2) hipLaunchKernelGGL(backward_pair_pack_kernel<2>, grid, dim3(256), 0, st, dev, plan->ix);
    else hipLaunchKernelGGL(backward_pair_pack_kernel<1>, grid, dim3(256), 0, st, dev, plan->ix);
    return check_launch();
}

int rrl_mlp_input_backward_multi(int n, const rrl_input_bwd_t* ps, void* stream) {
    if (!ps || n <= 0 || n > kMaxGroup) return RRL_EINVAL;
// ... 25 lines not shown
```

recovery_rl_amd/experiment.py:

```python
import datetime
import itertools
import os
import os.path as osp
import pickle
import time

import numpy as np
import torch

from . import distributed as dist_utils
from . import paths
from .env import make_env, make_vec_env, register_env
from .replay_memory import ConstraintReplayMemory, ReplayMemory
from .sac import SAC
from .fused import mlp3_supported
from .utils import linear_schedule, trace_range

STAT_KEYS = ("env_steps", "episodes", "num_viols", "viol_and_recovery", "viol_and_no_recovery",
             "num_successes", "recovery_steps", "constraint_steps", "sac_updates", "qrisk_updates")


def uses_constraint_buffer(cfg):
    return cfg.use_recovery or cfg.DGD_constraints or cfg.RCPO


def uses_mb_recovery(cfg):
    return cfg.use_recovery and not (cfg.MF_recovery or cfg.Q_sampling_recovery)


class VectorLoop:

    def __init__(self, cfg, env, agent, memory, recovery_memory, recovery_policy=None,
                 nu_schedule=None):
        self.cfg, self.env, self.agent = cfg, env, agent
        self.memory, self.recovery_memory = memory, recovery_memory
        self.recovery_policy = recovery_policy
        self.nu_schedule = nu_schedule or (lambda ep: cfg.nu)
        self.n = env.num_envs
        dev = env.device
        self.device = dev
        self.obs = None
        self.stats = torch.zeros(len(STAT_KEYS), dtype=torch.int64, device=dev)
        self.reward_sums = torch.zeros(2, dtype=torch.float64, device=dev)
        self.ep_reward = torch.zeros(self.n, dtype=torch.float32, device=dev)
        self.total_numsteps = 0
        self.updates = 0
        self.num_constraint_violations = 0
        self.graph = None
        self.host_updates = [0, 0]
        self._graph_updates = (0, 0)
        self._actor = None
        self.carry_actor = paths.switch("RRL_CARRY_ACTOR")
        self.draw_ahead = paths.switch("RRL_DRAW_AHEAD")
        fast = getattr(agent, "fast", None)
        self.sqrl_hip, self.sqrl_f16x3, self.qsample_hip, self.qsample_gated, self.qsample_f16x3 = paths.acting(
            cfg, fast is not None, fast is not None and fast.qrisk.w2p is not None)
        self._graph_ahead = False
        self.forget_plans = bool(recovery_policy is not None and self.n > 1 and hasattr(recovery_policy, "forget_plans")
                                 and not getattr(cfg, "keep_plan_warm_start", False))
        self._one = torch.ones((), dtype=torch.int64, device=dev)
        self.action_rng = torch.Generator(device=dev)
        self.action_rng.manual_seed(int(cfg.seed) + 0x5EED)
        self.episode_log = None
        self.step_outputs = False
        if self.n > 1 and hasattr(recovery_memory, "clamp_stratified"):
            recovery_memory.clamp_stratified = True

    def start(self):
        self.obs = self.env.reset()
        return self.obs

    def do_updates(self, i_episode=1, online_qrisk=True, rider=None):
        cfg = self.cfg
        fast = getattr(self.agent, "fast", None)
        qr = self.agent.safety_critic
        grouped = (fast is not None and fast.grouped and fast.sync_world == 1 and cfg.batch_size == fast.B
                   and hasattr(self.memory, "draw_desc")
                   and (not online_qrisk or qr.clamp_batch_size(cfg.batch_size, len(self.recovery_memory)) == fast.B))
        for u in range(cfg.updates_per_step):
            if grouped:
                with trace_range("sample+sac_update+qrisk_update"):
                    fast.update_pair(self.memory, self.recovery_memory if online_qrisk else None,
                                     rider=rider if u == cfg.updates_per_step - 1 else None,
                                     nu=self.nu_schedule(i_episode),
                                     draw_ahead=self.draw_ahead and cfg.updates_per_step == 1)
                self.host_updates[0] += 1
                if online_qrisk:
                    qr.updates += 1
                    qr.last_losses = (fast.losses[4], fast.losses[5], fast.losses[6] if qr.MF_recovery else None)
                    self.host_updates[1] += 1
                self.updates += 1
                continue
            assert rider is None
            with trace_range("sample+sac_update"):
                self.agent.update_parameters(self.memory, cfg.batch_size, self.updates,
                                             safety_critic=self.agent.safety_critic,
                                             nu=self.nu_schedule(i_episode))
            self.host_updates[0] += 1
            if online_qrisk:
                with trace_range("sample+qrisk_update"):
                    self.agent.safety_critic.update_parameters(memory=self.recovery_memory,
                                                               policy=self.agent.policy,
                                                               batch_size=cfg.batch_size, plot=0)
                self.host_updates[1] += 1
            self.updates += 1

    def sqrl_actor(self):
        if self._actor is None:
            from .fast_update import FastActor
            self._actor = FastActor(self.agent.fast, self.n)
            self._actor.sqrl_seed = int(self.cfg.seed) & 0xFFFFFFFFFFFFFFFF
            self._actor.sqrl_f16x3 = self.sqrl_f16x3
        return self._actor

    def qsample_actor(self):
        if self._actor is None:
            from .fast_update import FastActor
            self._actor = FastActor(self.agent.fast, self.n)
        self._actor.qsample_seed = int(self.cfg.seed) & 0xFFFFFFFFFFFFFFFF
        self._actor.qsample_f16x3 = self.qsample_f16x3
        return self._actor

    def act(self, obs, random_actions=False, train=True):
        cfg = self.cfg
        fast = getattr(self.agent, "fast", None)
        if self.qsample_hip and train and not random_actions and obs.shape[0] == self.n:
            return self.qsample_actor().act_qsample(obs, cfg.eps_safe, gated=self.qsample_gated)
        if self.sqrl_hip and train and not random_actions and obs.shape[0] == self.n:
            action = self.sqrl_actor().act_sqrl(obs, cfg.eps_safe)
            return action, action, None
        if (fast is not None and train and not random_actions and obs.shape[0] == self.n
                and (not cfg.use_recovery or cfg.MF_recovery) and not cfg.use_constraint_sampling):
            if self._actor is None:
                from .fast_update import FastActor
                self._actor = FastActor(fast, self.n)
            return self._actor.act(obs, cfg.eps_safe, cfg.use_recovery, cfg.MF_recovery,
                                   defer_select=fast.grouped and obs is self.env.obs and self._can_fuse_step())
        if random_actions:
            action = self.env.sample_actions() if self.n == 1 else self.env.sample_actions(generator=self.action_rng)
        elif (fast is not None and train and obs.shape[0] == self.n and uses_mb_recovery(cfg)
              and mlp3_supported(fast.policy.H, 2, 4) and mlp3_supported(fast.qrisk.H, 4, 1)):
            if self._actor is None:
                from .fast_update import FastActor
                self._actor = FastActor(fast, self.n)
            action, recovery = self._actor.act_gate(obs, cfg.eps_safe)
            rec_action = self.recovery_policy.act(obs, 0, mask=recovery)
            real_action = torch.where(recovery.bool().unsqueeze(1), rec_action, action)
            return action, real_action, recovery
        else:
            eps = self._policy_eps(self.agent.policy, obs) if self.n > 1 else None
            action = self.agent.select_action(obs, eval=not train) if eps is None else \
                self.agent.select_action(obs, eval=not train, eps=eps)
        if not cfg.use_recovery:
            return action, action, None
        risk = self.agent.safety_critic.get_value(obs, action).squeeze(1)
        recovery = risk > cfg.eps_safe
        if self.n == 1 and not bool(recovery[0].item()):
            return action, action.clone(), recovery
        if cfg.MF_recovery or cfg.Q_sampling_recovery:
            qr = self.agent.safety_critic
            eps = self._policy_eps(qr.policy, obs) if (cfg.MF_recovery and self.n > 1) else None
            if random_actions and getattr(self, "qsample_gated", False):
                lo, hi = self.qsample_actor().qsample_box
                cand = lo + (hi - lo) * torch.rand(obs.shape[0], 1000, lo.numel(), device=self.device, generator=self.action_rng)
                rec_action = qr.select_action(obs, candidates=cand)
            else:
                rec_action = qr.select_action(obs) if eps is None else qr.select_action(obs, eps=eps)
        else:
# ... 968 lines not shown
```

recovery_rl_amd/fast_update.py:

```python
import math

import ctypes as C

import torch

from . import _lib, paths
from .fused import NN, NT, TN, gemm, mlp3_forward, mlp3_supported
from .paths import (BASELINE_FLAGS, eval_qsample_f16x3_enabled, eval_qsample_line, eval_rollout_path,
                    eval_scoring, eval_sqrl_f16x3_enabled, eval_sqrl_line, fast_baselines_enabled, fast_eval_enabled,
                    fast_eval_maze_enabled, fast_eval_qsample_enabled, fast_eval_sqrl_enabled, fast_path_supported,
                    fast_qsample_enabled, fast_sqrl_enabled, pack_qsample_enabled, pack_sqrl_enabled, qsample_acting_path,
                    qsample_f16x3_enabled, qsample_scoring, sqrl_acting_path, sqrl_f16x3_enabled, sqrl_scoring,
                    uses_baseline_terms)


_TAPE = None


def set_tape(tape):
    global _TAPE
    _TAPE = tape


def record(kind, *payload):
# ... 191 lines not shown
                         finalize=self.finalize)
            if self.split and not self.finalize:
                self.parts = (self.scratch, self.nsplit, self.scratch.stride(0))
            return self.parts
        xg = x.unsqueeze(0).expand(G, -1, -1)
        gemm(NT, xg, P["W1"], out=self.h1, bias=P["b1"], relu=True)
        gemm(NT, self.h1, P["W2"], out=self.h2, bias=P["b2"], relu=True)
        gemm(NT, self.h2, P["W3"], out=self.out, bias=P["b3"])
        return self.parts

    def forward_desc(self, x, params=None, save=True, in_head=None):
        assert mlp3_supported(self.net.H, self.net.din, self.net.dout) and not self.finalize
        P = (params or self.net).p
        net = self.net
        self.x = x
        assert x.stride(1) == 1
        self.parts = (self.scratch, self.nsplit, self.scratch.stride(0)) if self.split else (self.out, 1, 0)
        p = _lib.ptr
        if in_head is not None:
            assert self.split and net.din == 4, "the input head lives in the column-split kernels"
        w2p = (params or self.net).w2_packed() if self.split else None
        return _lib.rrl_stack_t(net.G, x.shape[0], net.H, net.din, net.dout, x.stride(0), p(x), p(P["W1"]), p(P["b1"]),
                                p(P["W2"]), p(P["b2"]), p(P["W3"]), p(P["b3"]), p(self.h1) if save else None,
                                p(self.h2) if save else None, p(self.out), p(self.scratch) if self.split else None,
                                in_head if in_head is not None else _lib.rrl_policy_head_t(), int(in_head is not None),
                                p(w2p) if w2p is not None else None)

    def backward_descs(self, dout, weight_grads=True, input_grad=False):
        P, Gr, net = self.net.p, self.net.g, self.net
        G, B, H = net.G, self.B, net.H
        p = _lib.ptr
        wg = weight_grads
        if isinstance(dout, _lib.rrl_loss_t):
            loss = dout
        else:
            assert dout.is_contiguous()
            loss = _lib.rrl_loss_t(-1, 1, 0, p(dout), None, None, None, None, None, None, 0.0, 0, 0, 0, None, None, 0, 0, 0)
        head = _lib.rrl_head_bwd_t(loss, G, B, H, net.dout, p(self.h2), p(P["W3"]), p(Gr["W3"]) if wg else None,
                                   p(Gr["b3"]) if wg else None, p(self.dh2))
        if self.fuse_first:
            self._folded = bool(self.fold_dx and input_grad and loss.kind >= 0)
            first = _lib.rrl_first_layer_t(p(self.x), p(P["W1"]), self.x.stride(0), net.din,
                                           p(self.first_part) if wg else None, self.first_part.stride(0),
                                           p(self.dx_part) if input_grad else None, int(self._folded))
            hidden = _lib.rrl_hidden_bwd_t(G, B, H, p(self.dh2), p(self.h1), p(P["W2"]), p(Gr["W2"]) if wg else None,
                                           p(Gr["b2"]) if wg else None, None, first)
            return head, hidden, None
        hidden = _lib.rrl_hidden_bwd_t(G, B, H, p(self.dh2), p(self.h1), p(P["W2"]), p(Gr["W2"]) if wg else None,
                                       p(Gr["b2"]) if wg else None, p(self.dh1), _lib.rrl_first_layer_t())
        inp = _lib.rrl_input_bwd_t(G, B, H, net.din, self.x.stride(0), p(self.dh1), p(self.x), p(P["W1"]),
                                   p(Gr["W1"]) if wg else None, p(Gr["b1"]) if wg else None,
                                   p(self.dx) if input_grad else None)
        return head, hidden, inp

    def backward(self, dout, weight_grads=True, input_grad=False, fuse_loss=True):
        if not fuse_loss and isinstance(dout, _lib.rrl_loss_t):
            dout = loss_dout(dout, self.B, self.dOut)
        descs = self.backward_descs(dout, weight_grads, input_grad)
        if self.pair_hidden:
            backward_multi([descs])
        else:
            self._backward_gemm_reference(descs, weight_grads)
        if not input_grad:
            return None
        return self.dx_part if self.fuse_first else self.dx

    def _backward_gemm_reference(self, descs, weight_grads):
        head, _, inp = descs
        assert inp is not None, "the GEMM reference writes dh1: set_fuse_first(False)"
        lib, st, P, Gr = _lib.load(), _lib.current_stream(), self.net.p, self.net.g
        _lib.check(lib.rrl_mlp_head_backward_multi(1, C.byref(head), st), "rrl_mlp_head_backward_multi")
        if weight_grads:
            gemm(TN, self.dh2, self.h1, out=Gr["W2"], colsum=Gr["b2"])
        gemm(NN, self.dh2, P["W2"], out=self.dh1, mask=self.h1)
        _lib.check(lib.rrl_mlp_input_backward_multi(1, C.byref(inp), st), "rrl_mlp_input_backward_multi")


def forward_multi(descs):
    arr = (_lib.rrl_stack_t * len(descs))(*descs)
    record("forward", arr, len(descs))
    _lib.check(_lib.load().rrl_mlp3_forward_multi(len(descs), arr, _lib.current_stream()), "rrl_mlp3_forward_multi")


def backward_multi(triples):
    lib, st, n = _lib.load(), _lib.current_stream(), len(triples)
    head_list = [t[0] for t in triples]
    heads = (_lib.rrl_head_bwd_t * len(head_list))(*head_list)
    hidden = (_lib.rrl_hidden_bwd_t * n)(*[t[1] for t in triples])
    rest = [t[2] for t in triples if t[2] is not None]
    inputs = (_lib.rrl_input_bwd_t * len(rest))(*rest) if rest else None
    record("pair_bwd", heads, hidden, n)
    if inputs is not None:
        record("unsupported", "rrl_mlp_input_backward_multi")
    _lib.check(lib.rrl_mlp_backward_pair_multi(n, heads, hidden, st), "rrl_mlp_backward_pair_multi")
    if inputs is not None:
        _lib.check(lib.rrl_mlp_input_backward_multi(len(inputs), inputs, st), "rrl_mlp_input_backward_multi")


def heads_multi(heads):
    arr = (_lib.rrl_policy_head_t * len(heads))(*heads)
    record("heads", arr, len(heads))
    _lib.check(_lib.load().rrl_policy_heads_fwd_multi(len(heads), arr, _lib.current_stream()),
               "rrl_policy_heads_fwd_multi")


def loss_dout(loss, B, dout):
    assert loss.da_parts <= 1, "fuse_loss = False needs set_fuse_first(False)"
    _lib.check(_lib.load().rrl_loss_dout(C.byref(loss), B, dout.data_ptr(), _lib.current_stream()), "rrl_loss_dout")
    return dout


class StackRows(Stack):

    def __init__(self, parent, lo, hi):
        assert parent.net.G == 1, "row slices of a multi-head stack are not contiguous"
        self.parent, self.lo, self.hi = parent, lo, hi
        self.net, self.B = parent.net, hi - lo
        dev, H = parent.net.device, parent.net.H
        z = lambda *s: torch.empty(*s, dtype=torch.float32, device=dev)
        self.h1, self.h2 = parent.h1[:, lo:hi], parent.h2[:, lo:hi]
        self.dh1, self.dh2, self.dx = z(1, self.B, H), z(1, self.B, H), z(1, self.B, parent.net.din)
        self.dOut = z(1, self.B, parent.net.dout)
        self.pair_hidden = True
        self._folded = False
        self._init_first(dev, 1, self.B, H, parent.net.din)

    def forward(self, *a, **k):
        raise RuntimeError("run the parent's forward, then use .after_forward()")

    def after_forward(self):
        t, n_part, ps = self.parent.parts
        self.x = self.parent.x[self.lo:self.hi]
        self.parts = (t[0, 0, self.lo:self.hi] if n_part > 1 else t[0, self.lo:self.hi], n_part, ps)
        return self.parts


class FastUpdater:

    def __init__(self, agent, batch_size):
        self.agent = agent
        self.qr = agent.safety_critic
        self.B = B = batch_size
        dev = self.dev = agent.device
        self.lib = _lib.load()
        self.critic = flatten_twin_q(agent.critic, dev)
        self.critic_target = flatten_twin_q(agent.critic_target, dev)
        self.policy = flatten_policy(agent.policy, dev)
        self.qrisk = flatten_twin_q(self.qr.safety_critic, dev)
        self.qrisk_target = flatten_twin_q(self.qr.safety_critic_target, dev)
        self.recpolicy = flatten_policy(self.qr.policy, dev)
        z = lambda *s: torch.zeros(*s, dtype=torch.float32, device=dev)
        self.pol_a = Stack(self.policy, B)
        self.pol_ab = Stack(self.policy, 2 * B)
        self.pol_next, self.pol_b = StackRows(self.pol_ab, 0, B), StackRows(self.pol_ab, B, 2 * B)
        self.cri_a, self.cri_b = Stack(self.critic, B), Stack(self.critic, B)
        self.qr_a, self.qr_b = Stack(self.qrisk, B), Stack(self.qrisk, B)
        self.rec_a = Stack(self.recpolicy, B)
        self.cri_t, self.qr_t = Stack(self.critic, B), Stack(self.qrisk, B)
        self.grouped = all(mlp3_supported(net.H, net.din, net.dout)
                           for net in (self.critic, self.policy, self.qrisk, self.recpolicy))
        self.fuse_heads = True
        self.xu_q, self.x2u_q, self.xpu_q = z(B, 4), z(B, 4), z(B, 4)
        self.xu = z(B, 4)
        self.x_pol = z(2 * B, 4)
        self.x2u, self.xpu = self.x_pol[:B], self.x_pol[B:]
        self.logp2, self.logp = z(B), z(B)
        self.losses = z(8)
        self.sync_world, self._avg, self.sac_bucket = 1, None, None
        self.fuse_loss = True
        self._noise = None
        self.keyed = False
        self._noise_buf, self._actor_noise, self._actor_noise_fresh = None, None, False
        self.actor_rows = 0
        self.noise_seed = (int(getattr(agent, "seed", 0)) ^ 0x6E6F697365) & 0xFFFFFFFFFFFFFFFF
        self.noise_tick = torch.zeros(2, dtype=torch.int64, device=dev)
        self.alpha = torch.full((1,), float(agent.alpha), dtype=torch.float32, device=dev)
        self.scale = agent.policy.action_scale.to(dev).float().contiguous()
        self.bias = agent.policy.action_bias.to(dev).float().contiguous()
        self.rscale = self.qr.policy.action_scale.to(dev).float().contiguous()
        self.rbias = self.qr.policy.action_bias.to(dev).float().contiguous()
        self._init_baselines(agent, B, z)

    def _init_baselines(self, agent, B, z):
        dev = self.dev
        self.dgd, self.update_nu, self.rcpo = bool(agent.DGD_constraints), bool(agent.update_nu), bool(agent.RCPO)
        self.qr_p, self.qr_sa = Stack(self.qrisk, B), Stack(self.qrisk, B)
        self.penalty = z(B)
        self.dual_stats = z(4)
        if self.update_nu and not torch.is_tensor(agent.nu):
            agent.nu = torch.tensor(float(agent.nu), dtype=torch.float32, device=dev)
        if self.rcpo and not torch.is_tensor(agent.lambda_RCPO):
            agent.lambda_RCPO = torch.tensor(float(agent.lambda_RCPO), dtype=torch.float32, device=dev)
        if self.dgd:
            self._join_dx(self.cri_b, self.qr_p)
        for opt, prm, on in ((agent.nu_optim, agent.log_nu, self.update_nu),
                             (agent.lambda_RCPO_optim, agent.log_lambda_RCPO, self.rcpo)):
            if on:
                dual_state(opt, prm)

    def _join_dx(self, a, b):
        assert a.net.H == b.net.H and a.net.din == b.net.din and a.net.G == b.net.G == 2 and a.B == b.B
        if a.first_part is not None and not a.fold_dx:
            for st in (a, b):
                st.fuse_first, st.first_part, st.dx_part = False, None, None
        j = torch.zeros(4, a.B, a.net.din, dtype=torch.float32, device=self.dev)
        a.dx, b.dx = j[0:2], j[2:4]
        if a.dx_part is not None:
            jp = torch.zeros(2, *a.dx_part.shape, dtype=torch.float32, device=self.dev)
            a.dx_part, b.dx_part = jp[0], jp[1]

    def joint_d_action(self):
        a, b = self.cri_b, self.qr_p
        B, din = a.B, a.net.din
        if a.fuse_first:
            assert b.fuse_first and a._folded == b._folded
            n = a.dx_part.shape[0] // 4 if a._folded else a.dx_part.shape[0]
            assert 2 * n <= 16
            return (a.dx_part[0], 2 * n, B * din, 1), (2, a.dx_part.numel())
        return a.dx, (4, B * din)

    def _duals(self, nu):
        ag, p = self.agent, _lib.ptr
        out = []
        if self.dgd or self.update_nu:
            d = _lib.rrl_dual_t(stat=p(self.dual_stats[0:1]), eps_safe=float(ag.eps_safe), lr=float(0.1 * ag.lr))
            if self.update_nu:
                st = dual_state(ag.nu_optim, ag.log_nu)
                d.log_p, d.exp_avg, d.exp_avg_sq, d.step = p(ag.log_nu), p(st["exp_avg"]), p(st["exp_avg_sq"]), p(st["step"])
                d.value = p(ag.nu)
            if self.dgd:
                d.loss_in, d.loss_out, d.f_loss = p(self.losses[2:3]), p(self.dual_stats[2:3]), float(nu)
            out.append(d)
        if self.rcpo:
            st = dual_state(ag.lambda_RCPO_optim, ag.log_lambda_RCPO)
            out.append(_lib.rrl_dual_t(p(ag.log_lambda_RCPO), p(st["exp_avg"]), p(st["exp_avg_sq"]), p(st["step"]),
                                       p(ag.lambda_RCPO), p(self.dual_stats[1:2]), float(ag.eps_safe), float(0.1 * ag.lr),
                                       None, None, 0.0))
        return out

    def _penalty(self, z, want_penalty=True, mean=None):
        t, n_part, ps = z
        p = _lib.ptr
        a = _lib.rrl_penalty_args_t(self.B, p(t), n_part, ps, p(self.agent.lambda_RCPO) if want_penalty else None,
                                    p(self.penalty) if want_penalty else None, p(mean))
        record("penalty", a)
        _lib.check(self.lib.rrl_rcpo_penalty(C.byref(a), _lib.current_stream()), "rrl_rcpo_penalty")

    def policy_loss(self):
        return self.dual_stats[2] if self.dgd else self.losses[2]

    def stacks(self):
        return [self.pol_a, self.pol_ab, self.pol_next, self.pol_b, self.cri_a, self.cri_b, self.cri_t, self.qr_a,
                self.qr_b, self.qr_t, self.rec_a, self.qr_p, self.qr_sa]

# ... 38 lines not shown
            if isinstance(d_action, tuple):
                d_action, parts, ps, group = d_action
            da, ld, n_heads, hs = d_action[0, :, 2:4].data_ptr(), d_action.stride(1), 2, d_action.stride(0)
            if d_heads is not None:
                n_heads, hs = d_heads
        return _lib.rrl_loss_t(kind, n_part, part_stride, p(out), p(out_t), p(v0), p(v1), p(v2), p(v3), p(alpha),
                               float(f0), ld, n_heads, hs, da, p(loss), parts, ps, group)

    def _load_batch(self, batch, rows_loaded=False, rows=None):
        s, a, r, s2, m = batch
        if not rows_loaded:
            xu, x2u, xpu = rows or self.rows
            xu[:, 0:2] = s
            xu[:, 2:4] = a
            x2u[:, 0:2] = s2
            xpu[:, 0:2] = s
        return s, a, r.reshape(-1), s2, m.reshape(-1)

    @property
    def rows(self):
        return (self.xu, self.x2u, self.xpu)

    @property
    def rows_q(self):
        return (self.xu_q, self.x2u_q, self.xpu_q)

    def _noise_pairs(self):
        n_act, n_upd = self.actor_rows, 4 * self.B * 2
        need = n_upd + 2 * n_act * 2
        if self._noise_buf is None or self._noise_buf.numel() != need:
            self._noise_buf = torch.zeros(need, dtype=torch.float32, device=self.dev)
        self._noise = self._noise_buf[:n_upd].view(4, self.B, 2)
        self._actor_noise = self._noise_buf[n_upd:].view(2, n_act, 2) if n_act else None
        self._actor_noise_fresh = n_act > 0
        return need // 2

    def _fill_noise(self):
        pairs = self._noise_pairs()
        record("unsupported", "rrl_normal_fill")
        _lib.check(self.lib.rrl_normal_fill(pairs, self.noise_seed, 0, _lib.ptr(self.noise_tick), 1,
                                            _lib.ptr(self._noise_buf), _lib.current_stream()), "rrl_normal_fill")

    def noise(self, which):
        if which == 0 or self._noise is None:
            self._fill_noise()
        n = self._noise
        return (n[0], n[1]) if which == 0 else (n[2], n[3])

    def actor_noise(self, n):
        if self.actor_rows != n:
            self.actor_rows = n
            self._actor_noise_fresh = False
        if not self._actor_noise_fresh:
            self._fill_noise()
        self._actor_noise_fresh = False
        return self._actor_noise

    def _gauss_desc(self, head, eps, action_view, logp, n=None, obs_in=None, obs_out=None):
        t, n_part, ps = head
        p = _lib.ptr
        return _lib.rrl_policy_head_t(_lib.HEAD_GAUSS, n or self.B, p(t), n_part, ps, p(eps), p(self.scale),
                                      p(self.bias), p(action_view), action_view.stride(0), p(logp), None, p(obs_in),
                                      p(obs_out), None, 0.0)

    def _stoch_desc(self, head, eps, action_view, n=None):
        t, n_part, ps = head
        p = _lib.ptr
        return _lib.rrl_policy_head_t(_lib.HEAD_STOCH, n or self.B, p(t), n_part, ps, p(eps), p(self.rscale),
                                      p(self.rbias), p(action_view), action_view.stride(0), None, None, None, None,
                                      p(self.recpolicy.p["log_std"]), float(self.qr.policy.min_log_std))

    def can_draw_ahead(self):
        return bool(_TAPE is None and self.grouped and self.sync_world == 1 and self.B <= 256 and self.pol_ab.split
                    and self.policy.H == 256 and self.recpolicy.H == 256)

    def select_ahead(self, desc, memory, rows):
        d, _ = memory.draw_desc(self.B, rows=self.rows, ahead=rows)
        sel = _lib.rrl_draw_ahead_t(C.pointer(d), rows, _lib.ptr(memory.ahead_keys(self.B)))
        riders = _lib.rrl_fwd_riders_t(C.pointer(sel), None, None, 0, 0, 0, None, 0, None)
        _lib.check(self.lib.rrl_mlp3_forward_riders(C.byref(desc), C.byref(riders), _lib.current_stream()),
                   "rrl_mlp3_forward_riders")
        memory.ahead.selected(self.B, rows)

    def update_pair(self, memory, recovery_memory, rider=None, nu=None, draw_ahead=False):
        B, qr = self.B, self.qr
        ahead_ok = bool(draw_ahead and rider is not None and self.can_draw_ahead())
        keyed = memory.ahead.take(B) and ahead_ok
        rider_selects = ahead_ok and (keyed or not torch.cuda.is_current_stream_capturing())
        if rider is not None:
            rider[0].select_for = (memory, rider[0].n) if rider_selects and len(memory) + rider[0].n >= B else None
        self.keyed = keyed
        d1, batch = memory.draw_desc(B, rows=self.rows)
        d2 = batch_q = None
        if recovery_memory is not None:
            d2, batch_q = recovery_memory.draw_desc(B, pos_fraction=qr.pos_fraction, rows=self.rows_q,
                                                    demo_share=qr.demo_share)
        pairs = self._noise_pairs()
        if keyed:
            gat = _lib.rrl_draw_ahead_t(C.pointer(d1), 0, _lib.ptr(memory.ahead_keys(B)))
            riders = _lib.rrl_fwd_riders_t(None, C.pointer(gat), C.pointer(d2) if d2 is not None else None, pairs,
                                           self.noise_seed, 0, _lib.ptr(self.noise_tick), 1, _lib.ptr(self._noise_buf))
            desc = self.pol_ab.forward_desc(self.x_pol[:, 0:2])
            _lib.check(self.lib.rrl_mlp3_forward_riders(C.byref(desc), C.byref(riders), _lib.current_stream()),
                       "rrl_mlp3_forward_riders")
        else:
            record("sample", _lib.rrl_sample_args_t(C.pointer(d1), C.pointer(d2) if d2 is not None else None, pairs,
                                                    self.noise_seed, 0, _lib.ptr(self.noise_tick), 1,
                                                    _lib.ptr(self._noise_buf)), d1, d2)
            _lib.check(self.lib.rrl_sample_multi(C.byref(d1), C.byref(d2) if d2 is not None else None, pairs,
                                                 self.noise_seed, 0, _lib.ptr(self.noise_tick), 1,
                                                 _lib.ptr(self._noise_buf), _lib.current_stream()), "rrl_sample_multi")
        n = self._noise
        self.sac_update(batch, n[0], n[1], rows_loaded=True, nu=nu, grouped=True, policy_forwarded=keyed)
        if recovery_memory is not None:
            self.qrisk_update(batch_q, n[2], n[3], rows_loaded=True, rows=self.rows_q, grouped=True, rider=rider)
        return self.losses

    def _forwards(self, members, grouped, riders=()):
        if grouped and (len(members) + len(riders) > 1 or members[0][0].split):
            descs = list(riders) + [st.forward_desc(x, **opt) for st, x, opt in members]
            for k in range(0, len(descs), 4):
                forward_multi(descs[k:k + 4])
            return
        assert not riders
        for st, x, opt in members:
            assert opt.get("in_head") is None, "a policy head rides in the grouped column-split launches only"
            st.forward(x, params=opt.get("params"), save=opt.get("save", True))

    def _heads(self, heads, consumer, grouped):
        if grouped and self.fuse_heads and consumer.split:
            return heads
        live = [hd for hd in heads if hd is not None]
        if grouped:
            heads_multi(live)
        else:
            for hd in live:
                heads_multi([hd])
        return [None] * len(heads)

    def _backwards(self, members, grouped):
        if grouped and len(members) > 1:
            backward_multi([st.backward_descs(loss, wg, ig) for st, loss, wg, ig in members])
            return
        for st, loss, wg, ig in members:
            st.backward(loss, weight_grads=wg, input_grad=ig, fuse_loss=self.fuse_loss or grouped)

    def _nu(self, nu):
        if not self.dgd:
            return 0.0
        nu = self.agent.nu if nu is None else nu
        return float(nu)

    def sac_update(self, batch, eps_next, eps_pi, rows_loaded=False, nu=None, grouped=False, policy_forwarded=False):
        ag, B = self.agent, self.B
        nu = self._nu(nu)
        s, a, r, s2, m = self._load_batch(batch, rows_loaded)
        if not policy_forwarded:
            self._forwards([(self.pol_ab, self.x_pol[:, 0:2], {})], grouped)
        head2, head = self.pol_next.after_forward(), self.pol_b.after_forward()
        hd2, hd1 = self._heads([self._gauss_desc(head2, eps_next, self.x2u[:, 2:4], self.logp2),
                                self._gauss_desc(head, eps_pi, self.xpu[:, 2:4], self.logp)], self.cri_t, grouped)
        fwd = [(self.cri_t, self.x2u, dict(params=self.critic_target, save=False, in_head=hd2)),
               (self.cri_a, self.xu, {}), (self.cri_b, self.xpu, dict(in_head=hd1))]
        if self.dgd or self.update_nu:
            hq = None
            if hd1 is not None:
                hq = _lib.rrl_policy_head_t.from_buffer_copy(hd1)
                hq.action, hq.logp = None, None
            fwd.append((self.qr_p, self.xpu, dict(save=self.dgd, in_head=hq)))
        if self.rcpo:
            fwd.append((self.qr_sa, self.xu, dict(save=False)))
        self._forwards(fwd, grouped)
        qt, n_part, ps = self.cri_t.parts
        q, qp = self.cri_a.parts[0], self.cri_b.parts[0]
        if self.rcpo:
            self._penalty(self.qr_sa.parts, mean=self.dual_stats[1:2])
        if self.update_nu and not self.dgd:
            self._penalty(self.qr_p.parts, want_penalty=False, mean=self.dual_stats[0:1])
        members = [
            (self.cri_a, self._loss(_lib.LOSS_SAC_CRITIC, q, n_part, ps, out_t=qt, v0=self.logp2, v1=r, v2=m,
                                    v3=self.penalty if self.rcpo else None, alpha=self.alpha, f0=ag.gamma,
                                    loss=self.losses), True, False),
            (self.cri_b, self._loss(_lib.LOSS_SAC_POLICY, qp, n_part, ps, v0=self.logp, alpha=self.alpha,
                                    loss=self.losses[2:]), False, True)]
        if self.dgd:
            members.append((self.qr_p, self._loss(_lib.LOSS_DGD_QRISK, *self.qr_p.parts, f0=nu, loss=self.dual_stats[0:1]),
                            False, True))
        self._backwards(members, grouped)
        ht, hn, hs = head
        da, dh = self.joint_d_action() if self.dgd else (self.cri_b.dx_parts(), None)
        self._backwards([(self.pol_b, self._loss(_lib.LOSS_GAUSS_HEAD, ht, hn, hs, v0=eps_pi, v1=self.scale,
                                                 f0=float(ag.alpha) / B, d_action=da, d_heads=dh), True, False)], grouped)
        if self.sync_world > 1:
            self._sync(self.sac_bucket)
        adam_multi(ag.lr, [(self.critic, self.critic_target, ag.tau, self.cri_a.grad_part),
                           (self.policy, None, 0.0, self.pol_b.grad_part)], duals=self._duals(nu))
        return self.losses

    def can_carry_actor(self):
        return bool(self.grouped and self.qr.MF_recovery and self.fuse_heads and self.qr_t.split and self.qr_b.split
                    and self.pol_a.split and self.rec_a.split and self.sync_world == 1)

    def qrisk_update(self, batch, eps_next, eps_pi, rows_loaded=False, rows=None, grouped=False, rider=None):
        qr = self.qr
        xu, x2u, xpu = rows = rows or self.rows
        s, a, c, s2, m = self._load_batch(batch, rows_loaded, rows)
        mf = bool(qr.MF_recovery)
        assert rider is None or self.can_carry_actor()
        fwd = [(self.pol_a, x2u[:, 0:2], dict(save=False))]
        if mf:
            fwd.append((self.rec_a, xpu[:, 0:2], {}))
        self._forwards(fwd, grouped, riders=[rider[0].ride_policy(rider[1])] if rider else ())
        hd_next, hd_rec = self._heads([self._gauss_desc(self.pol_a.parts, eps_next, x2u[:, 2:4], self.logp2),
                                       self._stoch_desc(self.rec_a.parts, eps_pi, xpu[:, 2:4]) if mf else None],
                                      self.qr_t, grouped)
        self._forwards([(self.qr_t, x2u, dict(params=self.qrisk_target, save=False, in_head=hd_next)),
                        (self.qr_a, xu, {})], grouped)
        zt, n_part, ps = self.qr_t.parts
        z = self.qr_a.parts[0]
        self._backwards([(self.qr_a, self._loss(_lib.LOSS_QRISK_CRITIC, z, n_part, ps, out_t=zt, v0=c, v1=m,
                                                f0=qr.gamma_safe, loss=self.losses[4:]), True, False)], grouped)
        self._sync(self.qrisk.grad)
        self.qrisk.adam(qr.lr, target=self.qrisk_target, tau=qr.tau, part=self.qr_a.grad_part)
        if mf:
            raw, rn, rs = self.rec_a.parts
            ls = self.recpolicy.p["log_std"]
            self._forwards([(self.qr_b, xpu, dict(in_head=hd_rec))], grouped,
                           riders=[rider[0].ride_qrisk()] if rider else ())
            zp, n_part, ps = self.qr_b.parts
            self._backwards([(self.qr_b, self._loss(_lib.LOSS_QRISK_POLICY, zp, n_part, ps, loss=self.losses[6:]),
                              False, True)], grouped)
            self._backwards([(self.rec_a, self._loss(_lib.LOSS_STOCH_HEAD, raw, rn, rs, v0=eps_pi, v1=ls, v2=self.rscale,
                                                     f0=qr.policy.min_log_std, d_action=self.qr_b.dx_parts(),
                                                     loss=self.recpolicy.g["log_std"]), True, False)], grouped)
            self._sync(self.recpolicy.grad)
            self.recpolicy.adam(qr.lr, part=self.rec_a.grad_part)
        return self.losses


ACT_ENTRIES = {("sqrl", False, False): ("sqrl", "rrl_sqrl_act"),
               ("sqrl", False, True): ("sqrl_f16x3", "rrl_sqrl_act_f16x3"),
               ("qsample", False, False): ("qsample", "rrl_qsample_act"),
               ("qsample", True, False): ("qsample", "rrl_qsample_act_gated"),
               ("qsample", False, True): ("qsample_f16x3", "rrl_qsample_act_f16x3"),
               ("qsample", True, True): ("qsample_f16x3", "rrl_qsample_act_gated_f16x3")}
ACT_PACKED = {kind: entry.replace("_gated", "") + "_packed" for kind, entry in ACT_ENTRIES.values()}


class FastActor:

    def __init__(self, fast, n):
        self.f, self.n = fast, n
        dev = fast.dev
        z = lambda *s: torch.zeros(*s, dtype=torch.float32, device=dev)
        self.pol, self.qr, self.rec = Stack(fast.policy, n), Stack(fast.qrisk, n), Stack(fast.recpolicy, n)
        self.xa = z(n, 4)
        self.task_action, self.rec_action, self.real_action = z(n, 2), z(n, 2), z(n, 2)
        self.recovery = torch.zeros(n, dtype=torch.uint8, device=dev)
        self._ride = None
        self.select_for = None
        self.sqrl_seed = int(getattr(fast.agent, "seed", 0)) & 0xFFFFFFFFFFFFFFFF
        self.sqrl_tick = torch.zeros(2, dtype=torch.int64, device=dev)
        self.sqrl_f16x3 = False
        self.sqrl_w2h = None
        self.qsample_seed = self.sqrl_seed
        self.qsample_tick = torch.zeros(2, dtype=torch.int64, device=dev)
        ac = getattr(fast.qr, "ac_space", None)
        self.qsample_box = None if ac is None else tuple(
            torch.as_tensor(b, dtype=torch.float32, device=dev).contiguous() for b in (ac.low, ac.high))
        self._qsample_scratch = None
        self.qsample_f16x3 = False
# ... 277 lines not shown
```

recovery_rl_amd/paths.py:

```python
import os
from collections import namedtuple

Switch = namedtuple("Switch", "name rule read doc")

ON, NOT_OFF, SET = '== "1"', '!= "0"', 'not in ("", "0")'
_RULES = {ON: lambda v: v == "1", NOT_OFF: lambda v: v != "0", SET: lambda v: v not in ("", "0")}
IMPORT, LOOP, EXPERIMENT, CALL = "import", "loop build", "Experiment build", "each call"

SWITCHES = (
    Switch("RRL_FAST_BASELINES", ON, CALL, "The comparison algorithms (LR, RSPO, SQRL, RCPO) take the fused update path too."),
    Switch("RRL_FAST_SQRL", ON, LOOP, "SQRL's constraint-sampling acting pass runs on the rrl_sqrl_act kernel (sqrl_acting_path)."),
    Switch("RRL_PACK_SQRL", ON, CALL, "--seeds_per_gpu packs SQRL, its acting pass as one rrl_sqrl_act_packed launch (read in "
           "experiment.run_packed; needs sqrl_acting_path(cfg) == \"hip\" and at most 8 seeds)."),
    Switch("RRL_SQRL_F16X3", ON, LOOP, "The rrl_sqrl_act pass scores its candidates with layer 2 of Q_risk in f16x3 "
           "(rrl_sqrl_act_f16x3); it matters only where sqrl_acting_path(cfg) == \"hip\"."),
    Switch("RRL_FAST_QSAMPLE", ON, LOOP, "The acting pass of --Q_sampling_recovery runs on the rrl_qsample_act kernels "
           "(qsample_acting_path)."),
    Switch("RRL_PACK_QSAMPLE", ON, LOOP, "That pass evaluates the recovery gate inside the qsample call (rrl_qsample_act_gated: "
           "three launches the tape records), and --seeds_per_gpu packs the line as one rrl_qsample_act_packed stage (read again in "
           "experiment.run_packed; needs qsample_acting_path(cfg) == \"hip\" and at most 8 seeds)."),
    Switch("RRL_QSAMPLE_F16X3", ON, LOOP, "The rrl_qsample_act pass scores its candidates with layer 2 of Q_risk in f16x3 "
           "(rrl_qsample_act_f16x3); only where qsample_acting_path(cfg) == \"hip\", and the random-action phase keeps its f32 code."),
    Switch("RRL_FAST_EVAL", ON, CALL, "Policy evaluation is one rrl_eval_rollout launch (eval_rollout_path, read at every evaluation)."),
    Switch("RRL_FAST_EVAL_MAZE", ON, CALL, "On top of RRL_FAST_EVAL=1: Maze evaluates on rrl_eval_rollout_maze."),
    Switch("RRL_FAST_EVAL_QSAMPLE", ON, CALL, "On top of RRL_FAST_EVAL=1: --Q_sampling_recovery evaluates on rrl_eval_rollout_qs, "
           "whatever RRL_FAST_QSAMPLE says."),
    Switch("RRL_FAST_EVAL_SQRL", ON, CALL, "On top of RRL_FAST_EVAL=1: --use_constraint_sampling evaluates on rrl_eval_rollout_sqrl, "
           "whatever RRL_FAST_SQRL says."),
    Switch("RRL_EVAL_SQRL_F16X3", ON, EXPERIMENT, "The SQRL evaluation scores its candidates in f16x3 (rrl_eval_rollout_sqrl_f16x3), "
           "independent of RRL_SQRL_F16X3; kept as Experiment.eval_f16x3_switches and used from then on."),
    Switch("RRL_EVAL_QSAMPLE_F16X3", ON, EXPERIMENT, "The Q-sampling evaluation scores its candidates in f16x3 "
           "(rrl_eval_rollout_qs_f16x3), independent of RRL_QSAMPLE_F16X3; kept as Experiment.eval_f16x3_switches likewise."),
    Switch("RRL_W2_FRAG", NOT_OFF, EXPERIMENT + " (FlatNet) and " + CALL + " (the path functions)", "The 256-wide nets keep W2 a "
           "second time in MFMA fragment order, which the acting kernels need; 0: A/B runs of profiles/."),
    Switch("RRL_CARRY_ACTOR", NOT_OFF, LOOP, "Two of the acting pass's forwards ride in the Q_risk update's launches; 0: the pass's "
           "own two launches (A/B and the bit-identity test)."),
    Switch("RRL_DRAW_AHEAD", NOT_OFF, LOOP, "The task batch's keys are selected one step ahead, without a draw launch "
           "(FastUpdater.update_pair); 0: off."),
    Switch("RRL_PLAN_F16X3", SET, CALL, "A FusedPlanner built without an explicit f16x3 evaluates the hidden layers as three f16 "
           "MFMA products of hi / lo splits."),
    Switch("RRL_ROCTX", SET, IMPORT, "roctx ranges around the stages of the lock-step iteration (utils.trace_range), for marker "
           "traces of the eager loop."),
    Switch("RRL_DIST_FORCE_INIT", SET, CALL, "distributed.init() makes a 1-rank process group, so that every collective really goes "
           "through the backend."),
)
_ROW = {s.name: s for s in SWITCHES}


def switch(name):
    return _RULES[_ROW[name].rule](os.environ.get(name, ""))


def _named(name):
    return lambda: switch(name)


fast_baselines_enabled = _named("RRL_FAST_BASELINES")
fast_sqrl_enabled, pack_sqrl_enabled, sqrl_f16x3_enabled = map(_named, ("RRL_FAST_SQRL", "RRL_PACK_SQRL", "RRL_SQRL_F16X3"))
fast_qsample_enabled, pack_qsample_enabled, qsample_f16x3_enabled = map(
    _named, ("RRL_FAST_QSAMPLE", "RRL_PACK_QSAMPLE", "RRL_QSAMPLE_F16X3"))
fast_eval_enabled, fast_eval_maze_enabled, fast_eval_qsample_enabled, fast_eval_sqrl_enabled = map(
    _named, ("RRL_FAST_EVAL", "RRL_FAST_EVAL_MAZE", "RRL_FAST_EVAL_QSAMPLE", "RRL_FAST_EVAL_SQRL"))
eval_sqrl_f16x3_enabled, eval_qsample_f16x3_enabled = map(_named, ("RRL_EVAL_SQRL_F16X3", "RRL_EVAL_QSAMPLE_F16X3"))


BASELINE_FLAGS = ("DGD_constraints", "update_nu", "nu_schedule", "use_constraint_sampling", "RCPO")


def uses_baseline_terms(cfg):
    return any(bool(getattr(cfg, f, False)) for f in BASELINE_FLAGS)


def fast_path_supported(cfg):
    return (cfg.policy == "Gaussian" and not cfg.automatic_entropy_tuning
            and (switch("RRL_FAST_BASELINES") or not uses_baseline_terms(cfg))
            and cfg.target_update_interval == 1 and not getattr(cfg, "cnn", False))


def fused_256(cfg):
    return fast_path_supported(cfg) and not getattr(cfg, "no_fast_path", False) and int(cfg.hidden_size) == 256


def sqrl_line(cfg):
    return bool(cfg.use_constraint_sampling) and not cfg.use_recovery


def qsample_line(cfg):
    return (bool(cfg.use_recovery) and bool(getattr(cfg, "Q_sampling_recovery", False)) and not cfg.MF_recovery
            and not cfg.use_constraint_sampling)


eval_sqrl_line, eval_qsample_line = sqrl_line, qsample_line

FRAG_MAX_SEEDS = 8
_REST = " (Gaussian policy, fixed alpha, --target_update_interval 1, no --no_fast_path, RRL_W2_FRAG not 0)"
_SEEDS = (lambda cfg, S: S <= FRAG_MAX_SEEDS,
          "at most %(max)d seeds per GPU (its launch reads Q_risk's fragment-order W2 copy, which packed runs keep up to that many "
          "seeds; got %(S)d)")
SQRL_NEEDS = (
    (lambda cfg, S: switch("RRL_FAST_SQRL"), "the acting pass on the rrl_sqrl_act kernel: set RRL_FAST_SQRL=1"),
    (lambda cfg, S: switch("RRL_FAST_BASELINES"), "the fused update path: set RRL_FAST_BASELINES=1"),
    (lambda cfg, S: not cfg.use_recovery,
     "a run without a recovery policy (--use_recovery takes SQRL's acting pass through module code)"),
    (lambda cfg, S: int(cfg.hidden_size) == 256, "--hidden_size 256 (the kernel's Q_risk width; got %(hidden)d)"),
    (lambda cfg, S: sqrl_line(cfg) and fused_256(cfg) and switch("RRL_W2_FRAG"), "the acting pass on the rrl_sqrl_act kernel" + _REST),
    _SEEDS)
QSAMPLE_NEEDS = (
    (lambda cfg, S: switch("RRL_FAST_QSAMPLE"), "the acting pass on the rrl_qsample_act kernels: set RRL_FAST_QSAMPLE=1"),
    (lambda cfg, S: not cfg.MF_recovery,
     "a run without --MF_recovery (the model-free recovery policy wins over --Q_sampling_recovery, and packs without this switch)"),
    (lambda cfg, S: not cfg.use_constraint_sampling, "a run without --use_constraint_sampling (SQRL's acting pass is another one)"),
    (lambda cfg, S: int(cfg.hidden_size) == 256, "--hidden_size 256 (the kernels' Q_risk width; got %(hidden)d)"),
    (lambda cfg, S: qsample_line(cfg) and fused_256(cfg) and switch("RRL_W2_FRAG"),
     "the acting pass on the rrl_qsample_act kernels" + _REST),
    _SEEDS)
PACKED_SEED_LIMITS = tuple(
    (flag, what + " packs at most %d seeds per GPU: it reads the fragment-order W2 copy of Q_risk, which packed runs keep up to "
     "that many seeds only (got %d)")
    for flag, what in (("sqrl_hip", "SQRL's constraint-sampling acting pass (rrl_sqrl_act_packed)"),
                       ("qsample_hip", "the Q-sampling recovery acting pass (rrl_qsample_act_packed)")))

# ... 66 lines not shown
```

Measured before the change: 29.39 million.

## Rebalance opening launches: Q(s,a) into first forward, safety draw into critic backward

In the keyed draw-ahead iteration, the critic's Q(s,a) forward now runs inside the first policy-forward launch, gathering its inputs directly from replay keys. The safety buffer's draw moves out of that launch and into the critic's paired backward launch. The aim is to even out the critical path between the first two launches and drop one forward from the second group. The cost is new kernel variants and more conditional setup, and the new path applies only when several preconditions hold (split path, H=256, fused loss, no DGD/RCPO/nu update).

```diff
diff --git a/include/rrl_hip.h b/include/rrl_hip.h
--- a/include/rrl_hip.h
+++ b/include/rrl_hip.h
@@ -287,10 +287,13 @@
     float* noise_out;
 } rrl_fwd_riders_t;
 int rrl_mlp3_forward_riders(const rrl_stack_t* stack, const rrl_fwd_riders_t* riders, void* stream);
+int rrl_mlp3_forward_riders_group(int n, const rrl_stack_t* stacks, const rrl_fwd_riders_t* riders, void* stream);
 int rrl_mlp_head_backward_multi(int n, const rrl_head_bwd_t* members, void* stream);
 int rrl_mlp_hidden_backward_multi(int n, const rrl_hidden_bwd_t* members, void* stream);
 int rrl_mlp_input_backward_multi(int n, const rrl_input_bwd_t* members, void* stream);
 int rrl_mlp_backward_pair_multi(int n, const rrl_head_bwd_t* heads, const rrl_hidden_bwd_t* hidden, void* stream);
+int rrl_mlp_backward_pair_draw(int n, const rrl_head_bwd_t* heads, const rrl_hidden_bwd_t* hidden, const rrl_draw_t* draw,
+                               void* stream);
 
 int rrl_loss_dout(const rrl_loss_t* loss, int B, float* dout, void* stream);
 typedef struct {
diff --git a/profiles/opening_launches_probe.py b/profiles/opening_launches_probe.py
--- /dev/null
+++ b/profiles/opening_launches_probe.py
@@ -0,0 +1,128 @@
+import ctypes as C
+import json
+import os
+import sys
+
+import torch
+
+ROOT = os.path.dirname(os.path.dirname(os.path.abspath(__file__)))
+sys.path.insert(0, ROOT)
+import bench
+from recovery_rl_amd import _lib
+from recovery_rl_amd.replay_memory import ConstraintReplayMemory, ReplayMemory
+
+DEV = torch.device("cuda:0")
+B, H, N_ENVS = 256, 256, 4096
+p = _lib.ptr
+
+
+def rows(n, gen):
+    f = lambda *s: torch.rand(*s, generator=gen, device=DEV)
+    return f(n, 2), f(n, 2), (f(n) < 0.1).float(), f(n, 2), f(n)
+
+
+def weights(gen, G, din, dout):
+    f = lambda *s: (torch.rand(*s, generator=gen, device=DEV) - 0.5) * 0.2
+    w = {"W1": f(G, H, din), "b1": f(G, H), "W2": f(G, H, H), "b2": f(G, H), "W3": f(G, dout, H), "b3": f(G, dout)}
+    w["w2p"] = torch.empty(G * H * H, device=DEV)
+    _lib.check(_lib.load().rrl_w2_pack(G, H, p(w["W2"]), p(w["w2p"]), _lib.current_stream()), "rrl_w2_pack")
+    return w
+
+
+def stack(w, M, x, save=True):
+    G, din, dout = w["W1"].shape[0], w["W1"].shape[2], w["W3"].shape[1]
+    z = lambda *s: torch.zeros(*s, device=DEV)
+    t = {"h1": z(G, M, H), "h2": z(G, M, H), "out": z(G, M, dout), "scratch": z(4, G, M, dout)}
+    desc = _lib.rrl_stack_t(G, M, H, din, dout, x.stride(0), p(x), p(w["W1"]), p(w["b1"]), p(w["W2"]), p(w["b2"]), p(w["W3"]),
+                            p(w["b3"]), p(t["h1"]) if save else None, p(t["h2"]) if save else None, p(t["out"]), p(t["scratch"]),
+                            _lib.rrl_policy_head_t(), 0, p(w["w2p"]))
+    return desc, t
+
+
+def backward(gen, keep):
+    r = lambda *s: torch.randn(*s, generator=gen, device=DEV)
+    z = lambda *s: torch.zeros(*s, device=DEV)
+    t = {"z": r(2, B, 1), "h2": r(2, B, H).relu(), "h1": r(2, B, H).relu(), "W3": r(2, 1, H) * 0.1, "W2": r(2, H, H) * 0.1,
+         "dW3": z(2, 1, H), "db3": z(2, 1), "dW2": z(2, H, H), "db2": z(2, H), "dh1": z(2, B, H), "dh2": z(2, B, H), "loss": z(2)}
+    keep.append(t)
+    loss = _lib.rrl_loss_t(_lib.LOSS_QRISK_POLICY, 1, 0, p(t["z"]), None, None, None, None, None, None, 0.0, 0, 0, 0, None,
+                           p(t["loss"]), 0, 0, 0)
+    head = _lib.rrl_head_bwd_t(loss, 2, B, H, 1, p(t["h2"]), p(t["W3"]), p(t["dW3"]), p(t["db3"]), p(t["dh2"]))
+    hidden = _lib.rrl_hidden_bwd_t(2, B, H, p(t["dh2"]), p(t["h1"]), p(t["W2"]), p(t["dW2"]), p(t["db2"]), p(t["dh1"]),
+                                   _lib.rrl_first_layer_t())
+    return head, hidden
+
+
+def main():
+    lib = _lib.load()
+    gen = torch.Generator(device=DEV).manual_seed(1)
+    memory = ReplayMemory(1000000, 5, device=DEV)
+    for _ in range(8):
+        memory.push(*rows(N_ENVS, gen))
+    safety = ConstraintReplayMemory(1000000, 5, device=DEV)
+    safety.push(*rows(20000, gen))
+    safety.pin()
+    for _ in range(8):
+        safety.push(*rows(N_ENVS, gen))
+    z = lambda *s: torch.zeros(*s, device=DEV)
+    xu, x_pol, rows_q = z(B, 4), z(2 * B, 4), (z(B, 4), z(B, 4), z(B, 4))
+    d1, _ = memory.draw_desc(B, rows=(xu, x_pol[:B], x_pol[B:]))
+    sel = _lib.rrl_draw_ahead_t(C.pointer(d1), 0, p(memory.ahead_keys(B)))
+    _lib.check(lib.rrl_draw_select(C.byref(sel), _lib.current_stream()), "rrl_draw_select")
+    d1.counter_inc = 0
+    gat = _lib.rrl_draw_ahead_t(C.pointer(d1), 0, p(memory.ahead_keys(B)))
+    d2, _ = safety.draw_desc(B, rows=rows_q, demo_share=0.5)
+    pairs = (4 * B * 2 + 2 * N_ENVS * 2) // 2
+    noise, ntick = z(2 * pairs), torch.zeros(2, dtype=torch.int64, device=DEV)
+
+    def riders(second):
+        return _lib.rrl_fwd_riders_t(None, C.pointer(gat), C.pointer(second) if second is not None else None, pairs, 77, 0,
+                                     p(ntick), 1, p(noise))
+    wp, wq = weights(gen, 1, 2, 4), weights(gen, 2, 4, 1)
+    pol, _tp = stack(wp, 2 * B, x_pol)
+    cri, _tq = stack(wq, B, xu)
+    with_draw, without = riders(d2), riders(None)
+    group = (_lib.rrl_stack_t * 2)(pol, cri)
+    xs = [torch.rand(B, 4, generator=gen, device=DEV) for _ in range(3)]
+    twins = [stack(wq, B, x, save=k > 0) for k, x in enumerate(xs)]
+    three = (_lib.rrl_stack_t * 3)(*[d for d, _ in twins])
+    two = (_lib.rrl_stack_t * 2)(*[d for d, _ in twins[:2]])
+    keep = []
+    members = [backward(gen, keep) for _ in range(2)]
+    heads = (_lib.rrl_head_bwd_t * 2)(*[m[0] for m in members])
+    hidden = (_lib.rrl_hidden_bwd_t * 2)(*[m[1] for m in members])
+    st = _lib.current_stream
+    launches = [
+        ("a_keyed_first_launch", lambda: lib.rrl_mlp3_forward_riders(C.byref(pol), C.byref(with_draw), st())),
+        ("b_without_safety_draw", lambda: lib.rrl_mlp3_forward_riders(C.byref(pol), C.byref(without), st())),
+        ("c_safety_draw_alone", lambda: lib.rrl_sample_multi(C.byref(d2), None, 0, 0, 0, None, 0, None, st())),
+        ("d_group_three_twins", lambda: lib.rrl_mlp3_forward_multi(3, three, st())),
+        ("d_group_two_twins", lambda: lib.rrl_mlp3_forward_multi(2, two, st())),
+        ("e_first_launch_with_q_sa", lambda: lib.rrl_mlp3_forward_riders_group(2, group, C.byref(without), st())),
+        ("e_first_launch_with_q_sa_and_draw", lambda: lib.rrl_mlp3_forward_riders_group(2, group, C.byref(with_draw), st())),
+        ("e_critic_backward", lambda: lib.rrl_mlp_backward_pair_multi(2, heads, hidden, st())),
+        ("e_critic_backward_with_draw", lambda: lib.rrl_mlp_backward_pair_draw(2, heads, hidden, C.byref(d2), st())),
+    ]
+    us = {}
+    for rep in range(3):
+        for name, launch in launches:
+            def checked(launch=launch, name=name):
+                _lib.check(launch(), name)
+            us.setdefault(name, []).append(round(bench._graph_of(checked, 50, DEV) * 1e6, 3))
+    torch.cuda.synchronize()
+    memory.check_error()
+    safety.check_error()
+    med = {k: sorted(v)[1] for k, v in us.items()}
+    out = {"what": "us per launch, 50 launches per captured graph, three passes (median below)", "us": us, "median_us": med,
+           "a_minus_b": round(med["a_keyed_first_launch"] - med["b_without_safety_draw"], 3),
+           "three_minus_two_twins": round(med["d_group_three_twins"] - med["d_group_two_twins"], 3),
+           "q_sa_in_first_launch": round(med["e_first_launch_with_q_sa"] - med["b_without_safety_draw"], 3),
+           "draw_in_critic_backward": round(med["e_critic_backward_with_draw"] - med["e_critic_backward"], 3)}
+    text = json.dumps(out, indent=1)
+    print(text)
+    if len(sys.argv) > 1:
+        open(sys.argv[1], "w").write(text + "\n")
+
+
+if __name__ == "__main__":
+    main()
diff --git a/recovery_rl_amd/_lib.py b/recovery_rl_amd/_lib.py
--- a/recovery_rl_amd/_lib.py
+++ b/recovery_rl_amd/_lib.py
@@ -27,6 +27,7 @@
     "rrl_nav_offline",
     "rrl_maze_step", "rrl_maze_reset", "rrl_maze_offline",
     "rrl_replay_push", "rrl_sample_multi", "rrl_draw_select", "rrl_mlp3_forward_riders",
+    "rrl_mlp3_forward_riders_group", "rrl_mlp_backward_pair_draw",
     "rrl_nav_step_push_x", "rrl_maze_step_push_x",
     "rrl_sample_multi_packed", "rrl_pack_clear", "rrl_mlp3_forward_multi_packed", "rrl_mlp_head_backward_multi_packed",
     "rrl_mlp_hidden_backward_multi_packed", "rrl_mlp_backward_pair_multi_packed", "rrl_adam_step_multi_packed", "rrl_nav_step_push_packed",
@@ -362,6 +363,8 @@
         "rrl_mlp3_forward_multi": (ci, [ci, C.POINTER(rrl_stack_t), vp]),
         "rrl_draw_select": (ci, [C.POINTER(rrl_draw_ahead_t), vp]),
         "rrl_mlp3_forward_riders": (ci, [C.POINTER(rrl_stack_t), C.POINTER(rrl_fwd_riders_t), vp]),
+        "rrl_mlp3_forward_riders_group": (ci, [ci, C.POINTER(rrl_stack_t), C.POINTER(rrl_fwd_riders_t), vp]),
+        "rrl_mlp_backward_pair_draw": (ci, [ci, C.POINTER(rrl_head_bwd_t), C.POINTER(rrl_hidden_bwd_t), C.POINTER(rrl_draw_t), vp]),
         "rrl_mlp_head_backward_multi": (ci, [ci, C.POINTER(rrl_head_bwd_t), vp]),
         "rrl_mlp_hidden_backward_multi": (ci, [ci, C.POINTER(rrl_hidden_bwd_t), vp]),
         "rrl_mlp_input_backward_multi": (ci, [ci, C.POINTER(rrl_input_bwd_t), vp]),
diff --git a/recovery_rl_amd/csrc/mlp_fwd_kernels.hip b/recovery_rl_amd/csrc/mlp_fwd_kernels.hip
--- a/recovery_rl_amd/csrc/mlp_fwd_kernels.hip
+++ b/recovery_rl_amd/csrc/mlp_fwd_kernels.hip
@@ -161,11 +161,15 @@
     int B;
     uint32_t last;
 };
-
-template <int R, int HC, bool LOOP = false, bool KEYED = false>
+struct RowKeyCols {
+    RowKeys rows;
+    const float* ac;
+};
+
+template <int R, int HC, bool LOOP = false, bool KEYED = false, bool KEYCOLS = false>
 __device__ __forceinline__ void mlp3_fwd_split_body(const StackArgs& a, float* partial, int bx, int g, int z, int G,
                                                     float* h1s, float* h2s, int nb = 1, int tiles = 1, float* xs_own = nullptr,
-                                                    const RowKeys* rk = nullptr) {
+                                                    const RowKeys* rk = nullptr, const float* key_ac = nullptr) {
     const int tid = threadIdx.x, lane = tid & 63;
     const int wave = __builtin_amdgcn_readfirstlane(tid >> 6);
     constexpr int kW = 4;
@@ -221,6 +225,23 @@
     const int blk0 = LOOP ? bx * nb : bx, blk1 = LOOP ? min(blk0 + nb, tiles) : bx + 1;
     const auto load_x = [&](int blk, float (&x)[R]) {
         const int i = lane & 15, q = lane >> 4, m0 = blk * (R * kStackRows);
+        if (KEYED && KEYCOLS && rk->keys) {
+            const float* lo = rk->lo;
+            const float* hi = rk->hi;
+            const float* ac = key_ac;
+            const uint32_t* keys = rk->keys;
+            rrl_pack::to_global_all(lo, hi, ac, keys);
+            const int col = min(q, din - 1);
+#pragma unroll
+            for (int t = 0; t < R; ++t) {
+                const int m = m0 + min(16 * t + i, M - 1 - m0);
+                const bool upper = m >= rk->B;
+                const unsigned e = 2u * min(keys[upper ? m - rk->B : m], rk->last) + unsigned(col & 1);
+                const float v_lo = lo[e], v_hi = hi[e], v_ac = ac[e];
+                x[t] = col >= 2 ? v_ac : upper ? v_hi : v_lo;
+            }
+            return;
+        }
         if (KEYED && rk->keys) {
             const float* lo = rk->lo;
             const float* hi = rk->hi;
@@ -550,6 +571,45 @@
     mlp3_fwd_split_body<R, 256, false, true>(a, partial, bx, rest % G, rest / G, G, lds, h2s, 1, 1, nullptr, &rk);
 }
 
+struct RiderGroup {
+    StackArgs a[2];
+    float* partial[2];
+    int G[2], tiles[2];
+    RowKeyCols rk[2];
+    int first1;
+};
+
+__global__ __launch_bounds__(256, 4) void mlp3_fwd_split_riders_group_kernel(RiderGroup rg, FwdRiders rd) {
+    extern __shared__ __attribute__((aligned(16))) float lds[];
+    const int x = blockIdx.x;
+    if (x < rd.n) {
+        char* smem = reinterpret_cast<char*>(lds);
+        if (x == rd.slot_sel)
+            select_ahead_body(rd.sel.rb, rd.sel.B, rd.sel.seed, rd.sel.counter, rd.sel.counter_dev, rd.sel.table_mask,
+                              rd.rows_ahead, rd.sel_keys, smem);
+        else if (x == rd.slot_gat)
+            gather_ahead_body(rd.gat.rb, rd.gat.B, rd.gat.counter, rd.gat.counter_dev, rd.gat.counter_inc, rd.gat_keys,
+                              rd.gat.out);
+        else if (x == rd.slot_second) draw_body(rd.second, smem);
+        else noise_body(rd.nz, x - rd.slot_noise);
+        return;
+    }
+    const int k = (x - rd.n) >= rg.first1;
+    StackArgs a = rg.a[k];
+    float* partial = rg.partial[k];
+    const RowKeys rk = rg.rk[k].rows;
+    const float* ac = rg.rk[k].ac;
+    const int G = rg.G[k], tiles = rg.tiles[k];
+    globalize(a);
+    rrl_pack::to_global(partial);
+    arrive_together(a.M, a.H, a.din, a.dout, a.ldx, a.use_in_head, a.in_head.kind, a.in_head.n_part, a.in_head.part_stride,
+                    a.in_head.ld_action, a.in_head.min_log_std, G, tiles, rk.B, rk.last);
+    const int local = x - rd.n - (k ? rg.first1 : 0);
+    const int bx = local % tiles, rest = local / tiles;
+    mlp3_fwd_split_body<1, 256, false, true, true>(a, partial, bx, rest % G, rest / G, G, lds,
+                                                   lds + kStackRows * (kStackMaxH + kSplitPad), 1, 1, nullptr, &rk, ac);
+}
+
 template <int R>
 __global__ __launch_bounds__(256, 4) void mlp3_fwd_split_pack_kernel(const StackGroup* __restrict__ groups, rrl_pack::Idx ix) {
     extern __shared__ __attribute__((aligned(16))) float lds[];
@@ -751,17 +811,11 @@
     return check_launch();
 }
 
-int rrl_mlp3_forward_riders(const rrl_stack_t* stack, const rrl_fwd_riders_t* riders, void* stream) {
-    if (!stack || !riders) return RRL_EINVAL;
-    StackGroup sg;
-    int path;
-    int rc = build_stack_group(1, stack, sg, path);
-    if (rc != RRL_OK) return rc;
-    if ((path != 0 && path != 3) || stack->H != 256) return RRL_EINVAL;
-    FwdRiders rd{};
-    RowKeys rk{};
+static int build_fwd_riders(const rrl_stack_t* stack, const rrl_fwd_riders_t* riders, FwdRiders& rd, RowKeys& rk, size_t& lds) {
+    rd = FwdRiders{};
+    rk = RowKeys{};
     rd.slot_sel = rd.slot_gat = rd.slot_second = rd.slot_noise = -1;
-    size_t lds = split_lds_floats(path == 0 ? 1 : kBigR) * 4;
+    int rc;
     const auto rider = [&](const rrl_draw_t* d, DrawArgs& a, int& slot) {
         int threads = 0;
         size_t l = 0;
@@ -798,6 +852,20 @@
         rd.n += rd.nz.blocks;
     }
     if (lds > 64 * 1024) return RRL_ERANGE;
+    return RRL_OK;
+}
+
+int rrl_mlp3_forward_riders(const rrl_stack_t* stack, const rrl_fwd_riders_t* riders, void* stream) {
+    if (!stack || !riders) return RRL_EINVAL;
+    StackGroup sg;
+    int path;
+    int rc = build_stack_group(1, stack, sg, path);
+    if (rc != RRL_OK) return rc;
+    if ((path != 0 && path != 3) || stack->H != 256) return RRL_EINVAL;
+    FwdRiders rd;
+    RowKeys rk;
+    size_t lds = split_lds_floats(path == 0 ? 1 : kBigR) * 4;
+    if ((rc = build_fwd_riders(stack, riders, rd, rk, lds)) != RRL_OK) return rc;
     const dim3 grid(unsigned(rd.n + sg.first[1]));
     hipStream_t s = (hipStream_t)stream;
     if (path == 0)
@@ -806,6 +874,38 @@
     else
         hipLaunchKernelGGL(mlp3_fwd_split_riders_kernel<kBigR>, grid, dim3(256), lds, s, sg.a[0], sg.partial[0], sg.G[0],
                            sg.tiles[0], rk, rd);
+    return check_launch();
+}
+
+int rrl_mlp3_forward_riders_group(int n, const rrl_stack_t* stacks, const rrl_fwd_riders_t* riders, void* stream) {
+    if (!stacks || !riders || n < 1 || n > 2) return RRL_EINVAL;
+    if (n == 1) return rrl_mlp3_forward_riders(stacks, riders, stream);
+    StackGroup sg;
+    int path;
+    int rc = build_stack_group(2, stacks, sg, path);
+    if (rc != RRL_OK) return rc;
+    if (path != 0 || stacks[0].H != 256 || stacks[1].H != 256) return RRL_EINVAL;
+    FwdRiders rd;
+    RowKeys rk;
+    size_t lds = split_lds_floats(1) * 4;
+    if ((rc = build_fwd_riders(&stacks[0], riders, rd, rk, lds)) != RRL_OK) return rc;
+    RiderGroup rg{};
+    for (int k = 0; k < 2; ++k) {
+        rg.a[k] = sg.a[k];
+        rg.partial[k] = sg.partial[k];
+        rg.G[k] = sg.G[k];
+        rg.tiles[k] = sg.tiles[k];
+    }
+    rg.first1 = sg.first[1];
+    if (rk.keys) {
+        const rrl_stack_t& q = stacks[1];
+        if (q.M != rd.gat.B || q.din != 4 || q.use_in_head || !rd.gat.out.xu || q.x != (const float*)rd.gat.out.xu || q.ldx != 4)
+            return RRL_EINVAL;
+        rg.rk[0] = RowKeyCols{rk, rd.gat.rb.a};
+        rg.rk[1] = RowKeyCols{RowKeys{rk.keys, rd.gat.rb.s, rd.gat.rb.s, q.M, rk.last}, rd.gat.rb.a};
+    }
+    const dim3 grid(unsigned(rd.n + sg.first[2]));
+    hipLaunchKernelGGL(mlp3_fwd_split_riders_group_kernel, grid, dim3(256), lds, (hipStream_t)stream, rg, rd);
     return check_launch();
 }
 
diff --git a/recovery_rl_amd/csrc/mlp_kernels.hip b/recovery_rl_amd/csrc/mlp_kernels.hip
--- a/recovery_rl_amd/csrc/mlp_kernels.hip
+++ b/recovery_rl_amd/csrc/mlp_kernels.hip
@@ -5,6 +5,7 @@
 #include <algorithm>
 
 #include "mlp_common.hpp"
+#include "replay_draw.hpp"
 
 namespace {
 
@@ -1110,8 +1111,8 @@
 }
 
 template <int DOUT>
-__device__ __forceinline__ void backward_pair_body(const PairJobs& pj, int x, float* smem) {
-    const int k = blockIdx.y, z = blockIdx.z;
+__device__ __forceinline__ void backward_pair_body(const PairJobs& pj, int x, float* smem, int z) {
+    const int k = blockIdx.y;
     HeadBwdArgs hb = pj.head[k];
     const int blocks_x = pj.blocks_x[k];
     globalize(hb);
@@ -1193,13 +1194,22 @@
 template <int DOUT>
 __global__ __launch_bounds__(256) void backward_pair_kernel(PairJobs pj) {
     __shared__ __attribute__((aligned(16))) float smem[pair_smem_floats<DOUT>()];
-    backward_pair_body<DOUT>(pj, blockIdx.x, smem);
+    backward_pair_body<DOUT>(pj, blockIdx.x, smem, blockIdx.z);
+}
+template <int DOUT>
+__global__ __launch_bounds__(256) void backward_pair_draw_kernel(PairJobs pj, DrawArgs dr) {
+    __shared__ __attribute__((aligned(16))) float smem[pair_smem_floats<DOUT>()];
+    if (blockIdx.z == 0) {
+        if (blockIdx.x == 0 && blockIdx.y == 0) draw_body(dr, reinterpret_cast<char*>(smem));
+        return;
+    }
+    backward_pair_body<DOUT>(pj, blockIdx.x, smem, blockIdx.z - 1);
 }
 template <int DOUT>
 __global__ __launch_bounds__(256) void backward_pair_pack_kernel(const PairJobs* __restrict__ groups, rrl_pack::Idx ix) {
     __shared__ __attribute__((aligned(16))) float smem[pair_smem_floats<DOUT>()];
     RRL_PACK_LOCATE(ix, groups, s, local);
-    backward_pair_body<DOUT>(groups[s], local, smem);
+    backward_pair_body<DOUT>(groups[s], local, smem, blockIdx.z);
 }
 
 template <int DOUT>
@@ -1671,6 +1681,29 @@
     return check_launch();
 }
 
+int rrl_mlp_backward_pair_draw(int n, const rrl_head_bwd_t* heads, const rrl_hidden_bwd_t* hidden, const rrl_draw_t* draw,
+                               void* stream) {
+    if (!draw) return rrl_mlp_backward_pair_multi(n, heads, hidden, stream);
+    PairJobs pj;
+    int most = 1, dout = 0;
+    bool pair = false;
+    int rc = build_pair_jobs(n, heads, hidden, pj, most, pair, dout);
+    if (rc != RRL_OK) return rc;
+    if (!pair) return RRL_EINVAL;
+    DrawArgs dr{};
+    int threads = 0;
+    size_t lds = 0;
+    if ((rc = draw_setup(*draw, dr, threads, lds)) != RRL_OK) return rc;
+    const size_t have = size_t(dout == 4 ? pair_smem_floats<4>() : dout == 2 ? pair_smem_floats<2>() : pair_smem_floats<1>()) * 4;
+    if (threads > 256 || lds > have) return RRL_ERANGE;
+    hipStream_t st = (hipStream_t)stream;
+    const dim3 grid(most, n, 4);
+    if (dout == 4) hipLaunchKernelGGL(backward_pair_draw_kernel<4>, grid, dim3(256), 0, st, pj, dr);
+    else if (dout == 2) hipLaunchKernelGGL(backward_pair_draw_kernel<2>, grid, dim3(256), 0, st, pj, dr);
+    else hipLaunchKernelGGL(backward_pair_draw_kernel<1>, grid, dim3(256), 0, st, pj, dr);
+    return check_launch();
+}
+
 static int head_pack_plan(const rrl_pack::Key& key, int S, const int* n, const rrl_head_bwd_t* const* members, hipStream_t st,
                           const rrl_pack::Plan*& plan) {
     std::vector<HeadBwdGroup> groups(S);
diff --git a/recovery_rl_amd/experiment.py b/recovery_rl_amd/experiment.py
--- a/recovery_rl_amd/experiment.py
+++ b/recovery_rl_amd/experiment.py
@@ -52,6 +52,7 @@
         self._actor = None
         self.carry_actor = paths.switch("RRL_CARRY_ACTOR")
         self.draw_ahead = paths.switch("RRL_DRAW_AHEAD")
+        self.spread_opening = not paths.switch("RRL_PLAIN_OPENING")
         fast = getattr(agent, "fast", None)
         self.sqrl_hip, self.sqrl_f16x3, self.qsample_hip, self.qsample_gated, self.qsample_f16x3 = paths.acting(
             cfg, fast is not None, fast is not None and fast.qrisk.w2p is not None)
@@ -83,7 +84,8 @@
                     fast.update_pair(self.memory, self.recovery_memory if online_qrisk else None,
                                      rider=rider if u == cfg.updates_per_step - 1 else None,
                                      nu=self.nu_schedule(i_episode),
-                                     draw_ahead=self.draw_ahead and cfg.updates_per_step == 1)
+                                     draw_ahead=self.draw_ahead and cfg.updates_per_step == 1,
+                                     spread_opening=self.spread_opening)
                 self.host_updates[0] += 1
                 if online_qrisk:
                     qr.updates += 1
diff --git a/recovery_rl_amd/fast_update.py b/recovery_rl_amd/fast_update.py
--- a/recovery_rl_amd/fast_update.py
+++ b/recovery_rl_amd/fast_update.py
@@ -297,7 +297,7 @@
     _lib.check(_lib.load().rrl_mlp3_forward_multi(len(descs), arr, _lib.current_stream()), "rrl_mlp3_forward_multi")
 
 
-def backward_multi(triples):
+def backward_multi(triples, draw=None):
     lib, st, n = _lib.load(), _lib.current_stream(), len(triples)
     head_list = [t[0] for t in triples]
     heads = (_lib.rrl_head_bwd_t * len(head_list))(*head_list)
@@ -307,6 +307,10 @@
     record("pair_bwd", heads, hidden, n)
     if inputs is not None:
         record("unsupported", "rrl_mlp_input_backward_multi")
+    if draw is not None:
+        assert _TAPE is None and inputs is None, "a draw rides in solo paired launches only"
+        _lib.check(lib.rrl_mlp_backward_pair_draw(n, heads, hidden, C.byref(draw), st), "rrl_mlp_backward_pair_draw")
+        return
     _lib.check(lib.rrl_mlp_backward_pair_multi(n, heads, hidden, st), "rrl_mlp_backward_pair_multi")
     if inputs is not None:
         _lib.check(lib.rrl_mlp_input_backward_multi(len(inputs), inputs, st), "rrl_mlp_input_backward_multi")
@@ -385,6 +389,7 @@
         self.fuse_loss = True
         self._noise = None
         self.keyed = False
+        self.safety_draw_in, self.q_sa_rode = None, False
         self._noise_buf, self._actor_noise, self._actor_noise_fresh = None, None, False
         self.actor_rows = 0
         self.noise_seed = (int(getattr(agent, "seed", 0)) ^ 0x6E6F697365) & 0xFFFFFFFFFFFFFFFF
@@ -589,7 +594,10 @@
                    "rrl_mlp3_forward_riders")
         memory.ahead.selected(self.B, rows)
 
-    def update_pair(self, memory, recovery_memory, rider=None, nu=None, draw_ahead=False):
+    def can_spread_opening(self):
+        return bool(self.cri_a.split and self.critic.H == 256 and self.cri_a.fuse_first and self.fuse_loss and self.B % 64 == 0)
+
+    def update_pair(self, memory, recovery_memory, rider=None, nu=None, draw_ahead=False, spread_opening=True):
         B, qr = self.B, self.qr
         ahead_ok = bool(draw_ahead and rider is not None and self.can_draw_ahead())
         keyed = memory.ahead.take(B) and ahead_ok
@@ -603,13 +611,24 @@
             d2, batch_q = recovery_memory.draw_desc(B, pos_fraction=qr.pos_fraction, rows=self.rows_q,
                                                     demo_share=qr.demo_share)
         pairs = self._noise_pairs()
+        spread = bool(keyed and spread_opening and self.can_spread_opening())
+        q_rides = spread and not (self.dgd or self.update_nu or self.rcpo)
+        late_draw = d2 if spread else None
+        self.q_sa_rode = q_rides
+        self.safety_draw_in = None if d2 is None else "critic_backward" if spread else "first_forward" if keyed else "draw_launch"
         if keyed:
             gat = _lib.rrl_draw_ahead_t(C.pointer(d1), 0, _lib.ptr(memory.ahead_keys(B)))
-            riders = _lib.rrl_fwd_riders_t(None, C.pointer(gat), C.pointer(d2) if d2 is not None else None, pairs,
+            second = d2 if late_draw is None else None
+            riders = _lib.rrl_fwd_riders_t(None, C.pointer(gat), C.pointer(second) if second is not None else None, pairs,
                                            self.noise_seed, 0, _lib.ptr(self.noise_tick), 1, _lib.ptr(self._noise_buf))
             desc = self.pol_ab.forward_desc(self.x_pol[:, 0:2])
-            _lib.check(self.lib.rrl_mlp3_forward_riders(C.byref(desc), C.byref(riders), _lib.current_stream()),
-                       "rrl_mlp3_forward_riders")
+            if q_rides:
+                descs = (_lib.rrl_stack_t * 2)(desc, self.cri_a.forward_desc(self.xu))
+                _lib.check(self.lib.rrl_mlp3_forward_riders_group(2, descs, C.byref(riders), _lib.current_stream()),
+                           "rrl_mlp3_forward_riders_group")
+            else:
+                _lib.check(self.lib.rrl_mlp3_forward_riders(C.byref(desc), C.byref(riders), _lib.current_stream()),
+                           "rrl_mlp3_forward_riders")
         else:
             record("sample", _lib.rrl_sample_args_t(C.pointer(d1), C.pointer(d2) if d2 is not None else None, pairs,
                                                     self.noise_seed, 0, _lib.ptr(self.noise_tick), 1,
@@ -618,7 +637,8 @@
                                                  self.noise_seed, 0, _lib.ptr(self.noise_tick), 1,
                                                  _lib.ptr(self._noise_buf), _lib.current_stream()), "rrl_sample_multi")
         n = self._noise
-        self.sac_update(batch, n[0], n[1], rows_loaded=True, nu=nu, grouped=True, policy_forwarded=keyed)
+        self.sac_update(batch, n[0], n[1], rows_loaded=True, nu=nu, grouped=True, policy_forwarded=keyed,
+                        critic_forwarded=q_rides, draw=late_draw)
         if recovery_memory is not None:
             self.qrisk_update(batch_q, n[2], n[3], rows_loaded=True, rows=self.rows_q, grouped=True, rider=rider)
         return self.losses
@@ -645,10 +665,11 @@
                 heads_multi([hd])
         return [None] * len(heads)
 
-    def _backwards(self, members, grouped):
-        if grouped and len(members) > 1:
-            backward_multi([st.backward_descs(loss, wg, ig) for st, loss, wg, ig in members])
+    def _backwards(self, members, grouped, draw=None):
+        if grouped and (len(members) > 1 or draw is not None):
+            backward_multi([st.backward_descs(loss, wg, ig) for st, loss, wg, ig in members], draw=draw)
             return
+        assert draw is None
         for st, loss, wg, ig in members:
             st.backward(loss, weight_grads=wg, input_grad=ig, fuse_loss=self.fuse_loss or grouped)
 
@@ -658,7 +679,8 @@
         nu = self.agent.nu if nu is None else nu
         return float(nu)
 
-    def sac_update(self, batch, eps_next, eps_pi, rows_loaded=False, nu=None, grouped=False, policy_forwarded=False):
+    def sac_update(self, batch, eps_next, eps_pi, rows_loaded=False, nu=None, grouped=False, policy_forwarded=False,
+                   critic_forwarded=False, draw=None):
         ag, B = self.agent, self.B
         nu = self._nu(nu)
         s, a, r, s2, m = self._load_batch(batch, rows_loaded)
@@ -669,6 +691,8 @@
                                 self._gauss_desc(head, eps_pi, self.xpu[:, 2:4], self.logp)], self.cri_t, grouped)
         fwd = [(self.cri_t, self.x2u, dict(params=self.critic_target, save=False, in_head=hd2)),
                (self.cri_a, self.xu, {}), (self.cri_b, self.xpu, dict(in_head=hd1))]
+        if critic_forwarded:
+            del fwd[1]
         if self.dgd or self.update_nu:
             hq = None
             if hd1 is not None:
@@ -693,7 +717,7 @@
         if self.dgd:
             members.append((self.qr_p, self._loss(_lib.LOSS_DGD_QRISK, *self.qr_p.parts, f0=nu, loss=self.dual_stats[0:1]),
                             False, True))
-        self._backwards(members, grouped)
+        self._backwards(members, grouped, draw=draw)
         ht, hn, hs = head
         da, dh = self.joint_d_action() if self.dgd else (self.cri_b.dx_parts(), None)
         self._backwards([(self.pol_b, self._loss(_lib.LOSS_GAUSS_HEAD, ht, hn, hs, v0=eps_pi, v1=self.scale,
diff --git a/recovery_rl_amd/paths.py b/recovery_rl_amd/paths.py
--- a/recovery_rl_amd/paths.py
+++ b/recovery_rl_amd/paths.py
@@ -37,6 +37,9 @@
            "own two launches (A/B and the bit-identity test)."),
     Switch("RRL_DRAW_AHEAD", NOT_OFF, LOOP, "The task batch's keys are selected one step ahead, without a draw launch "
            "(FastUpdater.update_pair); 0: off."),
+    Switch("RRL_PLAIN_OPENING", ON, LOOP, "The keyed iteration opens as it did before its first two launches were evened out: the "
+           "safety buffer's draw in the first policy forward's launch, Q(s, a) in the second forward's (FastUpdater.update_pair, "
+           "spread_opening; A/B runs and the bit-identity test)."),
     Switch("RRL_PLAN_F16X3", SET, CALL, "A FusedPlanner built without an explicit f16x3 evaluates the hidden layers as three f16 "
            "MFMA products of hi / lo splits."),
     Switch("RRL_ROCTX", SET, IMPORT, "roctx ranges around the stages of the lock-step iteration (utils.trace_range), for marker "
```

New measurement: 29.35 million. Within noise of the previous version (-0.1%).
